# Tcadart/pyLatticeDSO

Hardware: AMD Instinct MI355X
Metric: beams/s assembly+PCG-solve (higher is better)
Workload: dtype f64

## Files before the change

### include/pylattice_hip.h

```cpp
#ifndef PYLATTICE_HIP_H
#define PYLATTICE_HIP_H

#include <stdint.h>

#ifdef __cplusplus
extern "C" {
#endif

typedef struct pl_context *pl_handle;

typedef enum {
  PL_OK = 0,
  PL_ERR_ARG = -1,
  PL_ERR_HIP = -2,
  PL_ERR_STATE = -3,
  PL_ERR_NOCONV = -4,
  PL_ERR_NAN = -5,
  PL_ERR_NODEVICE = -6
} pl_status;

typedef struct {
  int64_t n_nodes;
  int64_t n_beams;
  const double *node_xyz;
// ... 90 lines not shown
int pl_ddm_set_geometry(pl_handle h, const double *node_xyz );

int pl_set_bc(pl_handle h, const uint8_t *fixed, const double *ubar, const double *f);

int pl_set_periodic(pl_handle h, const int32_t *master );

int pl_update_radii(pl_handle h, const double *beam_radius);
int pl_set_multiplicity(pl_handle h, const double *beam_mult );
int pl_update_segments(pl_handle h, const double *seg_len, const int32_t *seg_nsub);

int pl_assemble(pl_handle h);

int pl_assemble_bsr(pl_handle h, int with_bc, int64_t *n_block_rows, int64_t *n_blocks);
int pl_get_bsr(pl_handle h, int64_t *rowptr , int32_t *colidx , double *vals );

int pl_spmv(pl_handle h, const double *x, double *y);
int pl_spmv_free(pl_handle h, const double *x, double *y);
int pl_spmv_bsr(pl_handle h, const double *x, double *y);

int pl_solve(pl_handle h, double rtol, int32_t max_iter, double *u, pl_stats_t *stats);

int pl_reactions(pl_handle h, const double *u, double *R);

int pl_sens(pl_handle h, const double *u, const double *lam, double *dCdr);

int pl_node_mod(pl_handle h, const double *u, double *out);

int pl_stress(pl_handle h, const double *u , int32_t where,
              double *station ,
              double *peak );
int pl_stress_pnorm(pl_handle h, const double *u , int32_t where, double p, double *phi, double *sigma_max,
                    double *dphi_du , double *dphi_dr );

int pl_buckling(pl_handle h, const double *u , int32_t length, double k_eff, int32_t shear,
                double *util , double *n_axial , double *n_crit );
int pl_buckling_pnorm(pl_handle h, const double *u , int32_t length, double k_eff, int32_t shear, double p,
                      double *bp, double *util_max, double *dbp_du , double *dbp_dr );

int pl_energy(pl_handle h, const double *u, double *energy);

int pl_schur(pl_handle h, const int32_t *boundary_nodes, int32_t nb, double rtol, int32_t max_iter, double *S);

#define PL_MULTI_MAX 64
int pl_spmv_multi(pl_handle h, int32_t n_rhs, int masked, const double *x, double *y);
int pl_solve_multi(pl_handle h, int32_t n_rhs, const double *ubar, const double *f, double rtol, int32_t max_iter,
                   double *u, pl_stats_t *stats);
int pl_schur_block(pl_handle h, const int32_t *boundary_nodes, int32_t nb, double rtol, int32_t max_iter,
                   int32_t block, double *S);

int pl_geom_spmv_multi(pl_handle h, const double *u, int32_t n_rhs, int masked, const double *x, double *y);
int pl_buckling_modes(pl_handle h, const double *u , int32_t n_modes, int32_t n_sub,
                      double rtol, int32_t max_iter,
                      double tol, int32_t max_outer,
                      double *load_factor , double *modes ,
                      double *residual ,
                      int32_t *n_found, int32_t *outer_iterations);

int pl_schur_cells(const pl_opts_t *o, int32_t n_inst, int32_t n_nodes, int32_t n_beams,
                   const int32_t *beam_conn , int32_t nb,
                   const int32_t *boundary_nodes ,
                   const double *node_xyz , const double *beam_radius ,
                   const double *seg_len , const int32_t *seg_nsub ,
                   double *S , int32_t *info );

int pl_cells_recover(const pl_opts_t *o, int32_t n_inst, int32_t n_nodes, int32_t n_beams,
                     const int32_t *beam_conn , int32_t nb,
                     const int32_t *boundary_nodes ,
                     const double *node_xyz , const double *beam_radius ,
                     const double *seg_len , const int32_t *seg_nsub ,
                     const double *u_b ,
                     const double *lam_b ,
                     double *u_full ,
                     double *lam_full ,
                     double *sens ,
                     int32_t *info );

int pl_get_records(pl_handle h, double *rec);

int pl_debug_partition(pl_handle h, int32_t *tile_of_node, int32_t *agg_of_node, int32_t *local_agg_of_node,
                       uint8_t *eliminated);

int pl_time_kernel(pl_handle h, int which, int reps, double *avg_ms);
int pl_algorithmic_bytes(pl_handle h, double *out3);
int pl_forget_history(pl_handle h);

int pl_debug_spd_solve(int device, int32_t n, const double *A, const double *b, double *x, double *quad,
                       int32_t fp32_factor);

int pl_dist_unique_id_bytes(void);
int pl_dist_unique_id(void *id_out);
int pl_dist_loopback_id(void *id_out);
int pl_dist_abort(pl_handle h);
int pl_dist_init(pl_handle h, int rank, int world, const void *unique_id, const int32_t *shared_local,
                 const int32_t *shared_global, int32_t n_shared, int32_t n_shared_global);

typedef struct pl_lattice pl_lattice;
typedef struct {
  int64_t n_nodes, n_beams, n_cell_beam, n_cell_node, n_created;
} pl_lattice_info_t;
int pl_generate_lattice(int64_t n_cells, const double *cell_coord, const double *cell_size, const double *cell_radii,
                        int32_t n_geom, int32_t n_tmpl, const double *tmpl, const int32_t *tmpl_type,
                        pl_lattice **out, pl_lattice_info_t *info);
int pl_lattice_fetch(const pl_lattice *L, double *node_xyz, int32_t *beam_conn, double *beam_radius, int32_t *beam_type,
                     int32_t *beam_cell0, int64_t *cell_beam_ptr , int64_t *cell_beam_idx,
                     int64_t *cell_node_ptr , int64_t *cell_node_idx, int32_t *created_nodes,
                     int32_t *created_beam);
void pl_lattice_free(pl_lattice *L);

int pl_penalize(int64_t n_beams, const double *node_xyz, const int32_t *beam_conn, const double *lzone ,
                double mesh_size, double *seg_len , int32_t *seg_nsub , double *pen_xyz );

int pl_boundary_index(int64_t n_cells, const int64_t *cell_node_ptr, const int64_t *cell_node_idx, int64_t n_nodes,
                      const double *node_xyz, const double *cell_coord, const double *cell_size, int64_t *index_boundary,
                      int64_t *visit, int64_t *n_visit);

int pl_boundary_index_rows(int64_t n_cells, const int64_t *cell_node_ptr, const int64_t *cell_node_idx, int64_t n_nodes,
                           const double *node_xyz, const double *cell_coord, const double *cell_size,
                           int64_t *index_boundary, int64_t *visit, int64_t *n_visit);

int pl_dist_set_peers(pl_handle h, const int32_t *shared_peer );

#ifdef __cplusplus
}
#endif
#endif
```

### pylatticedso_amd/_capi.py

```python
from __future__ import annotations

import ctypes as C
import os

import numpy as np

from .timing import timing as _timing

_HERE = os.path.dirname(os.path.abspath(__file__))
LIB_PATH = os.environ.get("PYLATTICE_HIP_LIB") or os.path.join(_HERE, "libpylattice_hip.so")

PL_OK, PL_ERR_ARG, PL_ERR_HIP, PL_ERR_STATE, PL_ERR_NOCONV, PL_ERR_NAN, PL_ERR_NODEVICE = 0, -1, -2, -3, -4, -5, -6

EXPORTS = ["pl_default_opts", "pl_opts_size", "pl_stats_size", "pl_abi_version", "pl_last_error", "pl_version", "pl_lzone", "pl_create", "pl_create_ddm",
           "pl_ddm_set_preconditioner", "pl_ddm_set_geometry", "pl_ddm_update_matrices", "pl_destroy", "pl_set_bc", "pl_set_periodic",
           "pl_update_radii", "pl_set_multiplicity", "pl_update_segments", "pl_assemble", "pl_assemble_bsr", "pl_get_bsr", "pl_spmv",
           "pl_spmv_free", "pl_spmv_bsr", "pl_solve", "pl_reactions", "pl_sens", "pl_energy", "pl_node_mod", "pl_schur",
           "pl_stress", "pl_stress_pnorm", "pl_buckling", "pl_buckling_pnorm",
           "pl_spmv_multi", "pl_solve_multi", "pl_schur_block", "pl_geom_spmv_multi", "pl_buckling_modes",
           "pl_schur_cells", "pl_cells_recover", "pl_get_records", "pl_debug_partition", "pl_time_kernel", "pl_algorithmic_bytes", "pl_forget_history", "pl_debug_spd_solve", "pl_dist_unique_id_bytes",
           "pl_dist_unique_id", "pl_dist_loopback_id", "pl_dist_abort", "pl_dist_init", "pl_dist_set_peers", "pl_generate_lattice", "pl_lattice_fetch",
           "pl_lattice_free", "pl_penalize", "pl_boundary_index", "pl_boundary_index_rows"]


class PlMesh(C.Structure):
    _fields_ = [("n_nodes", C.c_int64), ("n_beams", C.c_int64), ("node_xyz", C.c_void_p),
                ("beam_conn", C.c_void_p), ("beam_radius", C.c_void_p), ("seg_len", C.c_void_p),
                ("seg_nsub", C.c_void_p)]


class PlOpts(C.Structure):
    _fields_ = [("struct_size", C.c_uint32), ("abi_version", C.c_uint32),
                ("young", C.c_double), ("poisson", C.c_double), ("kappa", C.c_double), ("pen_coef", C.c_double),
                ("device", C.c_int32), ("spmv_kernel", C.c_int32), ("precond", C.c_int32), ("reorder", C.c_int32),
                ("check_every", C.c_int32), ("lanes_per_node", C.c_int32),
                ("tile_nodes", C.c_int32), ("coarse_max_dofs", C.c_int32), ("palette", C.c_int32),
                ("local_max_dofs", C.c_int32), ("precision", C.c_int32), ("restart_every", C.c_int32),
                ("alpha_max", C.c_double), ("grid_lo", C.c_double * 3), ("grid_hi", C.c_double * 3),
                ("grid_nodes", C.c_int64), ("mintol", C.c_double), ("compact_records", C.c_int32),
                ("condense", C.c_int32), ("chol_persistent", C.c_int32), ("cg_form", C.c_int32),
                ("tile_modes", C.c_int32), ("coarse_modes", C.c_int32), ("overlap", C.c_int32),
                ("coarse_storage", C.c_int32), ("warm_start", C.c_int32), ("short_iteration", C.c_int32)]


class PlStats(C.Structure):
    _fields_ = [("struct_size", C.c_uint32), ("iterations", C.c_int32), ("converged", C.c_int32),
                ("reserved_i", C.c_int32), ("rel_residual", C.c_double),
                ("b_norm", C.c_double), ("ms_assembly", C.c_double), ("ms_solve", C.c_double),
                ("ms_spmv_avg", C.c_double), ("precond_used", C.c_double), ("restarts", C.c_double),
                ("precision_used", C.c_double), ("info", C.c_double), ("stop_reason", C.c_double),
                ("condensed_nodes", C.c_double), ("cg_form_used", C.c_double), ("kp_form", C.c_double),
                ("comm_world", C.c_double), ("comm_rank", C.c_double), ("short_iteration_used", C.c_double),
                ("reserved", C.c_double * 2)]


class PlError(RuntimeError):
    def __init__(self, code, msg):
        super().__init__(f"libpylattice_hip error {code}: {msg}")
        self.code = code


_lib = None


def load_library(path: str | None = None):
    global _lib
    if _lib is not None and path is None:
        return _lib
    p = path or LIB_PATH
    if not os.path.exists(p):
        raise FileNotFoundError(f"{p} not found - build it with `make -C pylatticedso_amd/csrc` "
                                "(the HIP path has no CPU fallback)")
    lib = C.CDLL(p)
    lib.pl_last_error.restype = C.c_char_p
    lib.pl_version.restype = C.c_char_p
    lib.pl_destroy.restype = None
    for name in ("pl_opts_size", "pl_stats_size", "pl_abi_version"):
        getattr(lib, name).restype = C.c_uint32
    lib.pl_lattice_free.restype = None
    V, I32, I64, D = C.c_void_p, C.c_int32, C.c_int64, C.c_double
    sig = {"pl_default_opts": [V, C.c_uint32], "pl_opts_size": [], "pl_stats_size": [], "pl_abi_version": [], "pl_lzone": [I32, I64, I64, V, V, V, V], "pl_create": [V, V, V], "pl_create_ddm": [I64, I64, I32, V, I32, V, V, V, V],
           "pl_ddm_set_preconditioner": [V, I32, V, V], "pl_ddm_set_geometry": [V, V], "pl_ddm_update_matrices": [V, I32, V, V], "pl_destroy": [V], "pl_set_bc": [V, V, V, V], "pl_set_periodic": [V, V],
           "pl_update_radii": [V, V], "pl_set_multiplicity": [V, V], "pl_update_segments": [V, V, V], "pl_assemble": [V],
           "pl_assemble_bsr": [V, I32, V, V], "pl_get_bsr": [V, V, V, V], "pl_spmv": [V, V, V],
           "pl_spmv_free": [V, V, V], "pl_spmv_bsr": [V, V, V], "pl_solve": [V, D, I32, V, V],
           "pl_reactions": [V, V, V], "pl_sens": [V, V, V, V], "pl_energy": [V, V, V], "pl_node_mod": [V, V, V],
           "pl_stress": [V, V, I32, V, V], "pl_stress_pnorm": [V, V, I32, D, V, V, V, V],
           "pl_buckling": [V, V, I32, D, I32, V, V, V], "pl_buckling_pnorm": [V, V, I32, D, I32, D, V, V, V, V],
           "pl_schur": [V, V, I32, D, I32, V], "pl_spmv_multi": [V, I32, I32, V, V],
           "pl_solve_multi": [V, I32, V, V, D, I32, V, V], "pl_schur_block": [V, V, I32, D, I32, I32, V],
           "pl_geom_spmv_multi": [V, V, I32, I32, V, V],
           "pl_buckling_modes": [V, V, I32, I32, D, I32, D, I32, V, V, V, V, V],
           "pl_schur_cells": [V, I32, I32, I32, V, I32, V, V, V, V, V, V, V],
           "pl_cells_recover": [V, I32, I32, I32, V, I32, V, V, V, V, V, V, V, V, V, V, V],
           "pl_get_records": [V, V], "pl_debug_partition": [V, V, V, V, V], "pl_time_kernel": [V, I32, I32, V],
           "pl_algorithmic_bytes": [V, V], "pl_forget_history": [V], "pl_debug_spd_solve": [I32, I32, V, V, V, V, I32], "pl_dist_unique_id_bytes": [], "pl_dist_unique_id": [V], "pl_dist_loopback_id": [V], "pl_dist_abort": [V],
           "pl_dist_init": [V, I32, I32, V, V, V, I32, I32], "pl_dist_set_peers": [V, V],
           "pl_generate_lattice": [I64, V, V, V, I32, I32, V, V, V, V], "pl_lattice_fetch": [V] * 12,
           "pl_lattice_free": [V], "pl_penalize": [I64, V, V, V, D, V, V, V],
           "pl_boundary_index": [I64, V, V, I64, V, V, V, V, V, V],
           "pl_boundary_index_rows": [I64, V, V, I64, V, V, V, V, V, V]}
    for name, args in sig.items():
        getattr(lib, name).argtypes = args
    if lib.pl_opts_size() != C.sizeof(PlOpts) or lib.pl_stats_size() != C.sizeof(PlStats):
        raise ImportError(f"{p}: pl_opts_t / pl_stats_t are {lib.pl_opts_size()} / {lib.pl_stats_size()} bytes in the "
                          f"library, {C.sizeof(PlOpts)} / {C.sizeof(PlStats)} in this binding (ABI version "
                          f"{lib.pl_abi_version()}): rebuild libpylattice_hip.so")
    _lib = lib
    return lib


def default_opts(lib=None) -> "PlOpts":
    lib = lib or load_library()
    opts = PlOpts()
    _check(lib, lib.pl_default_opts(C.byref(opts), C.sizeof(PlOpts)))
    return opts


def _ptr(a):
    return None if a is None else a.ctypes.data_as(C.c_void_p)


def _f64(a, n=None):
    a = np.ascontiguousarray(a, dtype=np.float64)
    if n is not None and a.size != n:
        raise ValueError(f"expected {n} values, got {a.size}")
    return a


def _check(lib, rc, allow=()):
    if rc != PL_OK and rc not in allow:
        raise PlError(rc, lib.pl_last_error().decode())
    return rc


def lzone(node_xyz, beam_conn, beam_radius, device=0):
    lib = load_library()
    xyz = _f64(np.asarray(node_xyz).reshape(-1))
    conn = np.ascontiguousarray(beam_conn, dtype=np.int32).reshape(-1)
    rad = _f64(np.asarray(beam_radius).reshape(-1), len(conn) // 2)
    out = np.empty(len(conn), np.float64)
    _check(lib, lib.pl_lzone(int(device), len(xyz) // 3, len(conn) // 2, _ptr(xyz), _ptr(conn), _ptr(rad), _ptr(out)))
    return out.reshape(-1, 2)


def debug_spd_solve(A, b, device=0, fp32_factor=False):
    lib = load_library()
    A = np.ascontiguousarray(A, np.float64)
    b = np.ascontiguousarray(b, np.float64)
    x = np.empty_like(b)
    q = C.c_double()
    _check(lib, lib.pl_debug_spd_solve(device, len(b), _ptr(A), _ptr(b), _ptr(x), C.byref(q), int(bool(fp32_factor))))
    return x, q.value


MULTI_MAX = 64

SCHUR_CELLS_MAX_BOUNDARY, SCHUR_CELLS_MAX_INTERIOR, SCHUR_CELLS_MAX_BEAMS = 32, 16, 512


def schur_cells_fits(n_nodes, n_beams, n_boundary):
    return (0 < n_boundary <= SCHUR_CELLS_MAX_BOUNDARY and n_nodes - n_boundary <= SCHUR_CELLS_MAX_INTERIOR
            and 0 < n_beams <= SCHUR_CELLS_MAX_BEAMS)


def _per_instance(name, a, tail, n_inst):
    if a.shape == tail:
        a = np.broadcast_to(a, (n_inst,) + tail)
    elif a.shape != (n_inst,) + tail:
        raise ValueError(f"{name} must have shape {tail} or {(n_inst,) + tail}, got {a.shape}")
    return np.ascontiguousarray(a)


def schur_cells(node_xyz, beam_conn, boundary_nodes, beam_radius, seg_len, seg_nsub, young, poisson, kappa=0.9,
                pen_coef=1.5, device=0, n_inst=None):
    xyz, conn, bn, rad, slen, nsub, n_inst = _cell_batch_arrays(node_xyz, beam_conn, boundary_nodes, beam_radius, seg_len,
                                                                seg_nsub, n_inst)
    B, N = len(conn), xyz.shape[1]
    lib = load_library()
# ... 440 lines not shown
        return S

    def _columns(self, name, a, k=None):
        n6 = 6 * self.n_nodes
        a = np.asarray(a, dtype=np.float64)
        if a.shape in ((self.n_nodes, 6), (n6,)):
            a = a.reshape(1, n6)
        elif a.ndim == 3 and a.shape[1:] == (self.n_nodes, 6):
            a = a.reshape(a.shape[0], n6)
        elif not (a.ndim == 2 and a.shape[1] == n6):
            raise ValueError(f"{name} must have shape (k, {self.n_nodes}, 6) or (k, {n6}), got {a.shape}")
        if not 1 <= a.shape[0] <= MULTI_MAX:
            raise ValueError(f"{name}: 1 ... {MULTI_MAX} columns per call, got {a.shape[0]}")
        if k is not None and a.shape[0] != k:
            raise ValueError(f"{name} has {a.shape[0]} columns, {k} expected")
        return np.ascontiguousarray(a)

    def spmv_multi(self, X, masked=False):
        x = self._columns("X", X)
        y = np.empty_like(x)
        _check(self._lib, self._lib.pl_spmv_multi(self._h, x.shape[0], int(bool(masked)), _ptr(x), _ptr(y)))
        return y.reshape(x.shape[0], self.n_nodes, 6)

    def solve_multi(self, ubar=None, f=None, rtol=1e-8, max_iter=20000, raise_on_noconv=True):
        if ubar is None and f is None:
            raise ValueError("solve_multi needs ubar or f (they give the number of columns)")
        ub = None if ubar is None else self._columns("ubar", ubar)
        ff = None if f is None else self._columns("f", f, None if ub is None else ub.shape[0])
        k = (ub if ub is not None else ff).shape[0]
        u = np.empty((k, 6 * self.n_nodes), np.float64)
        st = (PlStats * k)()
        for s in st:
            s.struct_size = C.sizeof(PlStats)
        rc = self._lib.pl_solve_multi(self._h, k, _ptr(ub), _ptr(ff), float(rtol), int(max_iter), _ptr(u), st)
        keys = [n for n, _ in PlStats._fields_ if n not in ("reserved", "reserved_i", "struct_size")]
        stats = [{n: getattr(s, n) for n in keys} for s in st]
        if rc in (PL_OK, PL_ERR_NOCONV):
            _timing.device("pl_solve_multi: PCG (HIP events)", st[0].ms_solve)
        _check(self._lib, rc, allow=() if raise_on_noconv else (PL_ERR_NOCONV,))
        return u.reshape(k, self.n_nodes, 6), stats

    def geom_spmv_multi(self, X, u=None, masked=False):
        x = self._columns("X", X)
        u = None if u is None else _f64(np.asarray(u).reshape(-1), 6 * self.n_nodes)
        y = np.empty_like(x)
        _check(self._lib, self._lib.pl_geom_spmv_multi(self._h, _ptr(u), x.shape[0], int(bool(masked)), _ptr(x), _ptr(y)))
        return y.reshape(x.shape[0], self.n_nodes, 6)

    def buckling_modes(self, n_modes=4, u=None, n_sub=0, rtol=1e-10, max_iter=200000, tol=1e-9, max_outer=200,
                       raise_on_noconv=True):
        u = None if u is None else _f64(np.asarray(u).reshape(-1), 6 * self.n_nodes)
        n_modes = int(n_modes)
        lam = np.empty(max(n_modes, 0), np.float64)
        modes = np.empty((max(n_modes, 0), self.n_nodes, 6), np.float64)
        res = np.empty(max(n_modes, 0), np.float64)
        found, outer = C.c_int32(), C.c_int32()
        rc = self._lib.pl_buckling_modes(self._h, _ptr(u), n_modes, int(n_sub), float(rtol), int(max_iter), float(tol),
                                         int(max_outer), _ptr(lam), _ptr(modes), _ptr(res), C.byref(found), C.byref(outer))
        _check(self._lib, rc, allow=() if raise_on_noconv else (PL_ERR_NOCONV,))
        return {"load_factor": lam, "modes": modes, "residual": res, "n_found": found.value,
                "outer_iterations": outer.value}

    def geom_spmv_multi_host(self, X, u, masked=False, fixed=None):
        from . import geometric_host as GH
        if masked and fixed is None:
            raise ValueError("the masked product needs the mask given to set_bc")
        x = self._columns("X", X).reshape(-1, self.n_nodes, 6)
        return GH.geometric_apply(self.records(), self.beam_conn, u, x, fixed if masked else None)

    def buckling_modes_host(self, u, fixed, n_modes=4, n_sub=0, tol=1e-9, max_outer=200, dense=False):
        from . import geometric_host as GH
        rec = self.records()
        K = GH.elastic_matrix(rec, self.beam_conn, self.n_nodes)
        Kg = GH.geometric_matrix(rec, self.beam_conn, u, self.n_nodes)
        if dense:
            return GH.buckling_modes_dense(K, Kg, fixed, n_modes)
        return GH.buckling_modes_subspace(K, Kg, fixed, n_modes, n_sub, tol, max_outer)

    def time_kernel(self, which, reps=20):
        ms = C.c_double()
        _check(self._lib, self._lib.pl_time_kernel(self._h, int(which), int(reps), C.byref(ms)))
        return ms.value

    def algorithmic_bytes(self):
        out = (C.c_double * 3)()
        _check(self._lib, self._lib.pl_algorithmic_bytes(self._h, out))
        return {"spmv": out[0], "pcg_iter": out[1], "bsr": out[2]}

    def set_periodic(self, master):
        m = None if master is None else np.ascontiguousarray(master, dtype=np.int32)
        if m is not None and m.size != self.n_nodes:
            raise ValueError(f"expected {self.n_nodes} entries, got {m.size}")
        _check(self._lib, self._lib.pl_set_periodic(self._h, _ptr(m)))

    def forget_history(self):
        _check(self._lib, self._lib.pl_forget_history(self._h))

    @staticmethod
    def dist_unique_id() -> bytes:
        lib = load_library()
        n = lib.pl_dist_unique_id_bytes()
        buf = C.create_string_buffer(n)
        _check(lib, lib.pl_dist_unique_id(buf))
        return buf.raw

    @staticmethod
    def dist_loopback_id() -> bytes:
        lib = load_library()
        buf = C.create_string_buffer(lib.pl_dist_unique_id_bytes())
        _check(lib, lib.pl_dist_loopback_id(buf))
        return buf.raw

    def dist_abort(self):
        if getattr(self, "_h", None) is not None and self._h.value:
            self._lib.pl_dist_abort(self._h)

    def dist_init(self, rank, world, unique_id: bytes, shared_local, shared_global, n_shared_global, shared_peer=None):
        sl = np.ascontiguousarray(shared_local, dtype=np.int32)
        sg = np.ascontiguousarray(shared_global, dtype=np.int32)
        buf = C.create_string_buffer(unique_id, len(unique_id))
        _check(self._lib, self._lib.pl_dist_init(self._h, int(rank), int(world), buf, _ptr(sl), _ptr(sg),
                                                 int(len(sl)), int(n_shared_global)))
        if shared_peer is not None:
            sp = np.ascontiguousarray(shared_peer, dtype=np.int32)
            if sp.shape != sl.shape:
                raise ValueError("one peer rank per shared entry expected")
            _check(self._lib, self._lib.pl_dist_set_peers(self._h, _ptr(sp)))


for _name in ("assemble", "assemble_bsr", "get_bsr", "solve", "set_bc", "spmv", "spmv_free", "spmv_bsr", "reactions",
              "sens", "stress", "stress_pnorm", "buckling", "buckling_pnorm", "energy", "schur", "spmv_multi", "solve_multi", "geom_spmv_multi", "buckling_modes", "update_radii", "update_segments", "records"):
    _f = getattr(HipLattice, _name, None)
    if _f is not None:
        _f._timing_category = "hip"
        setattr(HipLattice, _name, _timing.timeit(_f))
```

### pylatticedso_amd/csrc/pl_api.hip

```cpp
#include "pl_solver.h"
#include "pl_condense.h"
#include "pl_multi.h"
#include "pl_stress.h"
#include "pl_buckling.h"
#include "pl_geom.h"


namespace {
template <typename WT>
int debug_spd_solve_t(int device, int32_t n, const double *A, const double *b, double *x, double *quad) {
  if (n <= 0 || !A || !b || !x) return fail(PL_ERR_ARG, "pl_debug_spd_solve: bad argument");
  int ndev = 0;
  if (hipGetDeviceCount(&ndev) != hipSuccess || ndev <= 0) return fail(PL_ERR_NODEVICE, "no HIP device visible");
  PL_HIP(hipSetDevice(device));
  const int np = (n + pl::kNB - 1) / pl::kNB * pl::kNB;
  std::vector<double> Ap((size_t)np * np, 0.0), bp(np, 0.0);
  for (int i = 0; i < np; ++i) {
    if (i < n) {
      std::memcpy(&Ap[(size_t)i * np], A + (size_t)i * n, n * sizeof(double));
      bp[i] = b[i];
    } else {
      Ap[(size_t)i * np + i] = 1.0;
    }
  }
// ... 756 lines not shown
    const size_t nn = (size_t)np * np;
    PL_HIP(h->dd_A.alloc(nn));
    PL_HIP(h->dd_Lf.alloc(nn));
    PL_HIP(h->dd_W.alloc(nn));
    PL_HIP(h->dd_Wt.alloc(nn));
    PL_HIP(h->dd_Dinv.alloc((size_t)np * pl::kNB));
    PL_HIP(h->dd_tv.alloc(np));
    PL_HIP(h->dd_info.alloc(2));
    PL_HIP(hipMemsetAsync(h->dd_W.p, 0, nn * sizeof(double), h->stream));
    PL_HIP(hipMemsetAsync(h->dd_Wt.p, 0, nn * sizeof(double), h->stream));
    h->dd_n = np;
  }
  h->dd_ready = false;
  PL_HIP(hipMemsetAsync(h->dd_A.p, 0, (size_t)np * np * sizeof(double), h->stream));
  PL_HIP(hipMemsetAsync(h->dd_info.p, 0, 2 * sizeof(int), h->stream));
  const int m = 6 * h->ddm_nb;
  const int64_t ne = h->ddm_cells * m * m;
  const uint8_t *fx = h->have_bc ? h->fixed.p : (const uint8_t *)nullptr;
  hipLaunchKernelGGL(pl::k_ddm_dense_assemble, dim3(grid_for(ne)), dim3(pl::kBlock), 0, h->stream, h->ddm_cells,
                     h->ddm_nb, h->ddm_cell_nodes.p, h->ddm_have_P ? h->ddm_cell_P.p : h->ddm_cell_S.p,
                     h->ddm_have_P ? h->ddm_Pt.p : h->ddm_St.p, fx, np, h->dd_A.p);
  hipLaunchKernelGGL(pl::k_ddm_dense_unit, dim3((np + 255) / 256), dim3(256), 0, h->stream, n6, np, fx, h->dd_A.p);
  pl::dense_factor_inverse(h->dd_A.p, h->dd_Lf.p, h->dd_W.p, h->dd_Wt.p, h->dd_Dinv.p, np, np, h->dd_info.p,
                           h->dd_bw, h->stream);
  PL_HIP(hipGetLastError());
  int info[2] = {0, 0};
  PL_HIP(hipMemcpyAsync(info, h->dd_info.p, sizeof(info), hipMemcpyDeviceToHost, h->stream));
  PL_HIP(hipStreamSynchronize(h->stream));
  h->dd_ready = (info[0] == 0);
  return PL_OK;
}

static int fem_factor_dense(pl_context *h) {
  const int64_t n6 = h->N * 6;
  const int np = (int)((n6 + pl::kNB - 1) / pl::kNB * pl::kNB);
  if (h->dd_n != np) {
    const size_t nn = (size_t)np * np;
    PL_HIP(h->dd_A.alloc(nn));
    PL_HIP(h->dd_Lf.alloc(nn));
    PL_HIP(h->dd_W.alloc(nn));
    PL_HIP(h->dd_Wt.alloc(nn));
    PL_HIP(h->dd_Dinv.alloc((size_t)np * pl::kNB));
    PL_HIP(h->dd_tv.alloc(np));
    PL_HIP(h->dd_info.alloc(2));
    PL_HIP(hipMemsetAsync(h->dd_W.p, 0, nn * sizeof(double), h->stream));
    PL_HIP(hipMemsetAsync(h->dd_Wt.p, 0, nn * sizeof(double), h->stream));
    h->dd_n = np;
    int64_t band = 0;
    for (int64_t i = 0; i < h->N; ++i)
      for (int64_t q = h->h_rowptr[i]; q < h->h_rowptr[i + 1]; ++q) band = std::max<int64_t>(band, std::llabs((long long)(h->h_col[q] - i)));
    h->dd_bw = (int)((6 * (band + 1) + pl::kNB - 1) / pl::kNB + 1);
  }
  h->dd_ready = false;
  int rc = ensure_bsr_buffers(h);
  if (rc) return rc;
  PL_HIP(hipMemsetAsync(h->dd_A.p, 0, (size_t)np * np * sizeof(double), h->stream));
  PL_HIP(hipMemsetAsync(h->dd_info.p, 0, 2 * sizeof(int), h->stream));
  rc = launch_bsr_fill(h, 1, h->stream);
  if (rc) return rc;
  h->have_bsr = false;
  hipLaunchKernelGGL(pl::k_bsr_to_dense, dim3(grid_for(h->nblk * 36)), dim3(pl::kBlock), 0, h->stream, h->N, h->nblk,
                     h->bsr_rowptr.p, h->bsr_col.p, (const double *)h->bsr_vals.p, np, h->dd_A.p);
  hipLaunchKernelGGL(pl::k_ddm_dense_unit, dim3((np + 255) / 256), dim3(256), 0, h->stream, n6, np, (const uint8_t *)nullptr,
                     h->dd_A.p);
  pl::dense_factor_inverse(h->dd_A.p, h->dd_Lf.p, h->dd_W.p, h->dd_Wt.p, h->dd_Dinv.p, np, np, h->dd_info.p, h->dd_bw,
                           h->stream);
  PL_HIP(hipGetLastError());
  int info[2] = {0, 0};
  PL_HIP(hipMemcpyAsync(info, h->dd_info.p, sizeof(info), hipMemcpyDeviceToHost, h->stream));
  PL_HIP(hipStreamSynchronize(h->stream));
  h->dd_ready = (info[0] == 0);
  if (h->dd_ready) PL_HIP(hipMemsetAsync(h->dinv.p, 0, n6 * sizeof(double), h->stream));
  return PL_OK;
}

void pl_destroy(pl_handle h) {
  if (!h) return;
  (void)hipSetDevice(h->opt.device);
  (void)hipStreamSynchronize(h->stream);
  if (h->comm_stream) (void)hipStreamSynchronize(h->comm_stream);
  pl::dist_destroy(h->dist);
  if (h->pal_host_flags != h->pal_fallback_flags) (void)hipHostFree(h->pal_host_flags);
  if (h->cls_host_flag) (void)hipHostFree(h->cls_host_flag);
  delete h;
}

int pl_set_bc(pl_handle h, const uint8_t *fixed, const double *ubar, const double *f) {
  if (!valid(h) || !fixed) return fail(PL_ERR_ARG, "pl_set_bc: null argument");
  PL_HIP(hipSetDevice(h->opt.device));
  const int64_t N = h->N;
  const size_t n6 = (size_t)N * 6;
  std::vector<uint8_t> fx(n6), bits(N);
  double *st = nullptr;
  if (int rcs = staging(h, &st)) return rcs;
  pl::parallel_for(N, [&](int64_t i0, int64_t i1, unsigned) {
    for (int64_t i = i0; i < i1; ++i) {
      const size_t src = 6 * (size_t)h->perm[i];
      uint8_t b = 0;
      for (int k = 0; k < 6; ++k) {
        const uint8_t v = fixed[src + k] ? 1 : 0;
        fx[6 * i + k] = v;
        b |= (uint8_t)(v << k);
        st[6 * i + k] = (ubar && v) ? ubar[src + k] : 0.0;
      }
      bits[i] = b;
    }
  }, 1 << 15);
  PL_HIP(hipMemcpyAsync(h->ubar.p, st, n6 * sizeof(double), hipMemcpyHostToDevice, h->stream));
  PL_HIP(hipMemcpyAsync(h->fixed.p, fx.data(), n6, hipMemcpyHostToDevice, h->stream));
  PL_HIP(hipMemcpyAsync(h->fixedbits.p, bits.data(), N, hipMemcpyHostToDevice, h->stream));
  PL_HIP(hipStreamSynchronize(h->stream));
  pl::parallel_for(N, [&](int64_t i0, int64_t i1, unsigned) {
    for (int64_t i = i0; i < i1; ++i) {
      const size_t src = 6 * (size_t)h->perm[i];
      for (int k = 0; k < 6; ++k) st[6 * i + k] = f ? f[src + k] : 0.0;
    }
  }, 1 << 15);
  PL_HIP(hipMemcpyAsync(h->f.p, st, n6 * sizeof(double), hipMemcpyHostToDevice, h->stream));
  PL_HIP(hipStreamSynchronize(h->stream));
  const bool same_mask = h->have_bc && !h->dist.active && h->h_fixedbits == bits;
  h->h_fixedbits = bits;
  if (same_mask) return PL_OK;
  h->have_bc = true;
  h->coarse.n_fix = -1;
  h->coarseL.n_fix = -1;
  {
    int rcs = select_condensed(h, bits);
    if (rcs) return rcs;
  }
  if (h->assembled && h->opkind == 1) {
    if (h->opt.precond >= 2 && h->opt.precond <= 4) {
      h->assembled = false;
      h->dd_ready = false;
      h->dd_blocks = false;
      h->dd2_ready = false;
    } else {
      pl::launch_invert_diag(h->N * 6, h->diag.p, h->fixed.p, h->dinv.p, h->stream);
      PL_HIP(hipStreamSynchronize(h->stream));
    }
  } else if (h->assembled) {
    int rc = launch_diag(h, h->stream);
    if (rc) return rc;
    rc = finish_diag_dist(h);
    if (rc) return rc;
    rc = launch_local_mask(h);
    if (rc) return rc;
    rc = launch_tile_blocks(h, h->stream);
    if (rc) return rc;
    rc = build_coarse(h);
    if (rc) return rc;
    rc = launch_dinv32(h);
    if (rc) return rc;
    rc = agree_condensed(h);
    if (rc) return rc;
    rc = launch_condensed_blocks(h, h->stream);
    if (rc) return rc;
    PL_HIP(hipStreamSynchronize(h->stream));
    {
      const bool keep = h->pal_ready;
      finish_condensed_classes(h);
      (void)keep;
    }
    if (h->bsr_with_bc) h->have_bsr = false;
    if (h->opt.precond == 5 && !h->dist.active) {
      rc = fem_factor_dense(h);
      if (rc) return rc;
    }
  }
  return PL_OK;
}

int pl_set_periodic(pl_handle h, const int32_t *master) {
  if (!valid(h)) return fail(PL_ERR_ARG, "pl_set_periodic: null handle");
  if (h->opkind != 0) return fail(PL_ERR_STATE, "pl_set_periodic: not available on a DDM handle");
  h->n_per_groups = 0;
  if (!master) return PL_OK;
  if (h->opt.precond != 1 || h->dist.active)
    return fail(PL_ERR_STATE, "pl_set_periodic: periodic constraints are served by the Jacobi PCG of a single-GPU handle (opts.precond = 1)");
  PL_HIP(hipSetDevice(h->opt.device));
  const int64_t N = h->N;
  std::vector<int32_t> inv((size_t)N);
  for (int64_t i = 0; i < N; ++i) inv[(size_t)h->perm[i]] = (int32_t)i;
  std::vector<int32_t> cnt((size_t)N, 0);
  for (int64_t i = 0; i < N; ++i) {
    const int32_t m = master[i];
    if (m < 0 || m >= N || master[m] != m) return fail(PL_ERR_ARG, "pl_set_periodic: master[i] must name a node that is its own master");
    cnt[(size_t)m]++;
  }
  std::vector<int32_t> ptr(1, 0), nodes, start((size_t)N, -1);
  for (int64_t m = 0; m < N; ++m)
    if (cnt[(size_t)m] >= 2) {
      start[(size_t)m] = (int32_t)ptr.size() - 1;
      ptr.push_back(ptr.back() + cnt[(size_t)m]);
    }
  nodes.resize((size_t)ptr.back());
  std::vector<int32_t> fill(ptr.begin(), ptr.end() - 1);
  for (int64_t i = 0; i < N; ++i) {
    const int32_t g = start[(size_t)master[i]];
    if (g >= 0) nodes[(size_t)fill[(size_t)g]++] = inv[(size_t)i];
  }
  const int64_t ng = (int64_t)ptr.size() - 1;
  if (ng == 0) return PL_OK;
  PL_HIP(h->per_ptr.alloc(ptr.size()));
  PL_HIP(h->per_nodes.alloc(nodes.size()));
  PL_HIP(hipMemcpy(h->per_ptr.p, ptr.data(), ptr.size() * sizeof(int32_t), hipMemcpyHostToDevice));
  PL_HIP(hipMemcpy(h->per_nodes.p, nodes.data(), nodes.size() * sizeof(int32_t), hipMemcpyHostToDevice));
  h->n_per_groups = ng;
  return PL_OK;
}

int pl_update_radii(pl_handle h, const double *beam_radius) {
  if (!valid(h) || !beam_radius) return fail(PL_ERR_ARG, "pl_update_radii: null argument");
  if (h->opkind != 0) return fail(PL_ERR_STATE, "pl_update_radii: not available on a DDM handle");
  for (int64_t b = 0; b < h->B; ++b)
    if (!(beam_radius[b] > 0.0)) return fail(PL_ERR_ARG, "pl_update_radii: non-positive radius");
  PL_HIP(hipSetDevice(h->opt.device));
  double *stg = nullptr;
  int rc = stagingB(h, &stg);
  if (rc) return rc;
  pl::parallel_for(h->B, [&](int64_t b0, int64_t b1, unsigned) {
    for (int64_t b = b0; b < b1; ++b) stg[b] = beam_radius[h->bperm[b]];
  }, 1 << 16);
  PL_HIP(hipMemcpyAsync(h->radius.p, stg, h->B * sizeof(double), hipMemcpyHostToDevice, h->stream));
  PL_HIP(hipStreamSynchronize(h->stream));
  h->assembled = false;
  h->have_bsr = false;
  return PL_OK;
}

int pl_set_multiplicity(pl_handle h, const double *beam_mult) {
  if (!valid(h)) return fail(PL_ERR_ARG, "pl_set_multiplicity: null handle");
  if (h->opkind != 0) return fail(PL_ERR_STATE, "pl_set_multiplicity: not available on a DDM handle");
  PL_HIP(hipSetDevice(h->opt.device));
  if (!beam_mult) {
    h->mult.release();
  } else {
    for (int64_t b = 0; b < h->B; ++b)
      if (!(beam_mult[b] > 0.0)) return fail(PL_ERR_ARG, "pl_set_multiplicity: non-positive multiplicity");
    std::vector<double> m(h->B);
    for (int64_t b = 0; b < h->B; ++b) m[b] = beam_mult[h->bperm[b]];
    if (!h->mult.p) PL_HIP(h->mult.alloc(h->B));
    PL_HIP(hipMemcpy(h->mult.p, m.data(), h->B * sizeof(double), hipMemcpyHostToDevice));
  }
  h->assembled = false;
  h->have_bsr = false;
  return PL_OK;
}

int pl_update_segments(pl_handle h, const double *seg_len, const int32_t *seg_nsub) {
  if (!valid(h) || !seg_len || !seg_nsub) return fail(PL_ERR_ARG, "pl_update_segments: null argument");
  PL_HIP(hipSetDevice(h->opt.device));
  std::vector<double> sl((size_t)h->B * 3);
  std::vector<int32_t> sn((size_t)h->B * 3);
  for (int64_t b = 0; b < h->B; ++b)
    for (int k = 0; k < 3; ++k) {
      sl[3 * b + k] = seg_len[3 * (size_t)h->bperm[b] + k];
      sn[3 * b + k] = seg_nsub[3 * (size_t)h->bperm[b] + k];
    }
  PL_HIP(hipMemcpy(h->seg_len.p, sl.data(), 3 * h->B * sizeof(double), hipMemcpyHostToDevice));
  PL_HIP(hipMemcpy(h->seg_nsub.p, sn.data(), 3 * h->B * sizeof(int32_t), hipMemcpyHostToDevice));
  h->assembled = false;
  h->have_bsr = false;
  return PL_OK;
}

int pl_assemble(pl_handle h) {
  if (!valid(h)) return fail(PL_ERR_ARG, "pl_assemble: null handle");
  PL_HIP(hipSetDevice(h->opt.device));
  if (h->opkind == 1) {
    if (h->assembled && (h->opt.precond == 0 || (h->opt.precond == 1 && !h->dd_ready && !h->dd_blocks) || h->dd_ready || h->dd_blocks)) {
      h->ms_assembly = 0.0;
      return PL_OK;
    }
    h->dd_ready = false;
    h->dd_blocks = false;
    h->dd2_ready = false;
    if (h->opt.precond == 4 && !h->dd2_plan)
      return fail(PL_ERR_STATE, "pl_assemble: precond = 4 on a DDM handle needs the node positions (pl_ddm_set_geometry)");
    if (h->opt.precond == 3 || h->opt.precond == 4) {
      PL_HIP(hipEventRecord(h->ev0, h->stream));
      if (!h->dd_B.p) PL_HIP(h->dd_B.alloc((size_t)h->N * 36));
      PL_HIP(hipMemsetAsync(h->dd_B.p, 0, (size_t)h->N * 36 * sizeof(double), h->stream));
      const int64_t ne = (int64_t)h->ddm_cells * h->ddm_nb * 36;
      hipLaunchKernelGGL(pl::k_ddm_node_blocks, dim3(grid_for(ne)), dim3(pl::kBlock), 0, h->stream, h->ddm_cells, h->ddm_nb,
                         h->ddm_cell_nodes.p, h->ddm_have_P ? h->ddm_cell_P.p : h->ddm_cell_S.p,
                         h->ddm_have_P ? h->ddm_Pt.p : h->ddm_St.p, h->dd_B.p);
      hipLaunchKernelGGL(pl::k_ddm_node_blocks_invert, dim3(grid_for(h->N)), dim3(pl::kBlock), 0, h->stream, h->N,
                         h->have_bc ? (const uint8_t *)h->fixed.p : (const uint8_t *)nullptr, h->dd_B.p);
      PL_HIP(hipMemsetAsync(h->dinv.p, 0, h->N * 6 * sizeof(double), h->stream));
      int info2[2] = {0, 0};
      if (h->opt.precond == 4) {
        pl::Coarse &cs = h->dd2;
        const int n = cs.ncp, m = 6 * h->ddm_nb;
        PL_HIP(hipMemsetAsync(cs.Ac, 0, (size_t)n * n * sizeof(double), h->stream));
        PL_HIP(hipMemsetAsync(cs.info, 0, 2 * sizeof(int), h->stream));
        hipLaunchKernelGGL(pl::k_ddm_coarse_cells, dim3((unsigned)h->ddm_cells), dim3(pl::kWave),
                           (size_t)2 * m * pl::kDdmModes * sizeof(double), h->stream, h->ddm_cells, h->ddm_nb,
                           h->ddm_cell_nodes.p, h->ddm_have_P ? h->ddm_cell_P.p : h->ddm_cell_S.p,
                           h->ddm_have_P ? h->ddm_Pt.p : h->ddm_St.p, h->dd2_agg.p, h->dd2_cen.p, h->dd2_xyz.p,
                           h->have_bc ? (const uint8_t *)h->fixed.p : (const uint8_t *)nullptr, n, cs.Ac);
        hipLaunchKernelGGL(pl::k_coarse_regularize, dim3((n + 255) / 256), dim3(256), 0, h->stream, n, cs.Ac);
        pl::TrtriPhases ph;
        ph.rows = 3;
        ph.stream = h->side2;
        ph.ev_go = h->ev_t0;
        ph.ev_done = h->ev_t1;
        pl::coarse_factor(cs, n, h->stream, nullptr, (unsigned *)nullptr, ph);
        cs.ainv_ready = false;
        if (cs.Ainv) {
          const long tiles = (long)(n / 32) * (n / 32 + 1) / 2;
          if (cs.w16)
            hipLaunchKernelGGL(pl::k_dense_explicit_inverse<pl::bf16_t>, dim3((unsigned)((tiles + 3) / 4)), dim3(256), 0,
                               h->stream, n, reinterpret_cast<const pl::bf16_t *>(cs.W), n, cs.Ainv);
          else
            hipLaunchKernelGGL(pl::k_dense_explicit_inverse<float>, dim3((unsigned)((tiles + 3) / 4)), dim3(256), 0, h->stream,
                               n, (const float *)cs.W, n, cs.Ainv);
          cs.ainv_ready = true;
        }
        PL_HIP(hipMemcpyAsync(info2, cs.info, sizeof(info2), hipMemcpyDeviceToHost, h->stream));
      }
      PL_HIP(hipEventRecord(h->ev1, h->stream));
      PL_HIP(hipEventSynchronize(h->ev1));
      PL_HIP(hipGetLastError());
      float ms = 0.f;
      PL_HIP(hipEventElapsedTime(&ms, h->ev0, h->ev1));
      h->ms_assembly = ms;
      h->dd2_ready = h->opt.precond == 4 && info2[0] == 0;
      h->dd_blocks = true;
      h->assembled = true;
      return PL_OK;
    }
    if (h->opt.precond == 2) {
      PL_HIP(hipEventRecord(h->ev0, h->stream));
      int rcp = ddm_factor_preconditioner(h);
      if (rcp) return rcp;
      if (h->dd_ready) {
        PL_HIP(hipMemsetAsync(h->dinv.p, 0, h->N * 6 * sizeof(double), h->stream));
        PL_HIP(hipEventRecord(h->ev1, h->stream));
        PL_HIP(hipEventSynchronize(h->ev1));
        float ms = 0.f;
        PL_HIP(hipEventElapsedTime(&ms, h->ev0, h->ev1));
        h->ms_assembly = ms;
        h->assembled = true;
        return PL_OK;
      }
    }
    if (h->opt.precond >= 1) {
      PL_HIP(hipMemsetAsync(h->diag.p, 0, h->N * 6 * sizeof(double), h->stream));
      const int64_t m = (int64_t)h->ddm_cells * h->ddm_nb * 6;
      hipLaunchKernelGGL(pl::k_ddm_diag, dim3(grid_for(m)), dim3(pl::kBlock), 0, h->stream, h->ddm_cells, h->ddm_nb,
                         h->ddm_cell_nodes.p, h->ddm_cell_S.p, h->ddm_St.p, h->diag.p);
    } else {
      pl::launch_fill(h->N * 6, 1.0, h->diag.p, h->stream);
    }
    pl::launch_invert_diag(h->N * 6, h->diag.p, h->have_bc ? h->fixed.p : nullptr, h->dinv.p, h->stream);
    PL_HIP(hipStreamSynchronize(h->stream));
    h->ms_assembly = 0.0;
    h->assembled = true;
    return PL_OK;
  }
  int rc = agree_condensed(h);
  if (rc) return rc;
  PL_HIP(hipEventRecord(h->ev0, h->stream));
  rc = launch_records(h);
  if (rc) return rc;
  rc = launch_local_mask(h);
  if (rc) return rc;
  PL_HIP(hipEventRecord(h->ev_fork, h->stream));
  PL_HIP(hipStreamWaitEvent(h->side, h->ev_fork, 0));
  rc = launch_palette(h, h->side);
  if (rc) return rc;
  rc = launch_diag(h, h->dist.active ? h->stream : h->side);
  if (rc) return rc;
  rc = finish_diag_dist(h);
  if (rc) return rc;
  rc = launch_tile_blocks(h, h->side);
  if (rc) return rc;
  rc = launch_condensed_blocks(h, h->side);
  if (rc) return rc;
  const bool refresh_bsr = h->want_bsr && (!h->bsr_with_bc || h->have_bc);
  int rc_fill = PL_OK;
  bool fill_queued = false;
  int64_t split = 0;
  if (refresh_bsr && h->side_cu && h->coarse.enabled && h->have_bc) {
    static const double kChainLinkMs = [] { const char *e = std::getenv("PL_CHAIN_LINK_MS"); return e ? std::atof(e) : 0.04; }();
    static const double kFillBlocksPerMs = [] { const char *e = std::getenv("PL_FILL_BLOCKS_PER_MS"); return e ? std::atof(e) : 8.5e6; }();
    const double chain_ms = kChainLinkMs * std::max(0, h->coarse.ncp / pl::kNB - 1);
    const double fit = chain_ms * kFillBlocksPerMs / std::max<double>(1.0, (double)h->nblk);
    split = fit >= 1.0 ? h->n_slices : (int64_t)(fit * (double)h->n_slices);
    if (split < h->n_slices / 16) split = 0;
  }
  bool part1_queued = false;
  auto queue_fill = [&](int phase) {
    if (!refresh_bsr || fill_queued) return;
    if (phase == 0) {
      if (split <= 0 || part1_queued) return;
      part1_queued = true;
      if (hipEventRecord(h->ev_chol, h->stream) != hipSuccess || hipStreamWaitEvent(h->side_cu, h->ev_chol, 0) != hipSuccess ||
          hipStreamWaitEvent(h->side_cu, h->ev_join, 0) != hipSuccess) {
        rc_fill = fail(PL_ERR_HIP, "pl_assemble: could not order the BSR fill beside the factorisation");
        return;
      }
      rc_fill = launch_bsr_fill(h, h->bsr_with_bc, h->side_cu, 0, split);
      if (hipEventRecord(h->ev_fill1, h->side_cu) != hipSuccess) rc_fill = fail(PL_ERR_HIP, "pl_assemble: event record failed");
      return;
    }
    fill_queued = true;
    if (hipEventRecord(h->ev_chol, h->stream) != hipSuccess || hipStreamWaitEvent(h->side, h->ev_chol, 0) != hipSuccess) {
      rc_fill = fail(PL_ERR_HIP, "pl_assemble: could not order the BSR fill behind the factorisation");
      return;
    }
    if (!rc_fill) rc_fill = launch_bsr_fill(h, h->bsr_with_bc, h->side, part1_queued ? split : 0, -1);
    if (part1_queued && hipStreamWaitEvent(h->side, h->ev_fill1, 0) != hipSuccess)
      rc_fill = fail(PL_ERR_HIP, "pl_assemble: event wait failed");
    if (hipEventRecord(h->ev_join, h->side) != hipSuccess) rc_fill = fail(PL_ERR_HIP, "pl_assemble: event record failed");
  };
  PL_HIP(hipEventRecord(h->ev_join, h->side));
  h->dd_ready = false;
  if (h->opt.precond == 5 && h->have_bc && !h->dist.active) {
    PL_HIP(hipStreamWaitEvent(h->stream, h->ev_join, 0));
    rc = fem_factor_dense(h);
    if (rc) return rc;
  }
  rc = build_coarse(h, h->coarse.enabled && h->have_bc ? std::function<void(int)>(queue_fill) : std::function<void(int)>());
  if (rc) return rc;
  queue_fill(1);
  if (rc_fill) return rc_fill;
  PL_HIP(hipStreamWaitEvent(h->stream, h->ev_join, 0));
  rc = launch_dinv32(h);
  if (rc) return rc;
  PL_HIP(hipEventRecord(h->ev1, h->stream));
  PL_HIP(hipStreamSynchronize(h->stream));
  finish_palette(h);
  finish_condensed_classes(h);
  for (pl::Coarse *cs : {&h->coarse, &h->coarseL})
    if (cs->ready && cs->Ac) {
      PL_HIP(hipMemsetAsync(cs->Ac, 0, (size_t)cs->ncp * cs->ncp * sizeof(double), h->stream));
      cs->ac_clean = true;
    }
  float ms = 0.f;
  PL_HIP(hipEventElapsedTime(&ms, h->ev0, h->ev1));
  h->ms_assembly = ms;
  h->assembled = true;
  h->have_bsr = refresh_bsr;
  return PL_OK;
}

int pl_assemble_bsr(pl_handle h, int with_bc, int64_t *n_block_rows, int64_t *n_blocks) {
  if (!valid(h)) return fail(PL_ERR_ARG, "pl_assemble_bsr: null handle");
  if (h->opkind != 0) return fail(PL_ERR_STATE, "pl_assemble_bsr: not available on a DDM handle");
  if (!h->assembled) return fail(PL_ERR_STATE, "pl_assemble_bsr: call pl_assemble first");
  if (with_bc && !h->have_bc) return fail(PL_ERR_STATE, "pl_assemble_bsr: with_bc needs pl_set_bc");
  PL_HIP(hipSetDevice(h->opt.device));
  if (int rcb = ensure_bsr_buffers(h)) return rcb;
  const bool fresh = h->have_bsr && h->want_bsr && h->bsr_with_bc == (with_bc ? 1 : 0);
  h->want_bsr = true;
  h->bsr_with_bc = with_bc ? 1 : 0;
  if (fresh) {
    if (n_block_rows) *n_block_rows = h->N;
    if (n_blocks) *n_blocks = h->nblk;
    return PL_OK;
  }
  PL_HIP(hipEventRecord(h->ev0, h->stream));
  int rc = launch_bsr_fill(h, with_bc, h->stream);
  if (rc) return rc;
  PL_HIP(hipEventRecord(h->ev1, h->stream));
  PL_HIP(hipStreamSynchronize(h->stream));
  float ms = 0.f;
  PL_HIP(hipEventElapsedTime(&ms, h->ev0, h->ev1));
  h->ms_assembly += ms;
  h->have_bsr = true;
  if (n_block_rows) *n_block_rows = h->N;
  if (n_blocks) *n_blocks = h->nblk;
  return PL_OK;
}

int pl_get_bsr(pl_handle h, int64_t *rowptr, int32_t *colidx, double *vals) {
  if (!valid(h)) return fail(PL_ERR_ARG, "pl_get_bsr: null handle");
  if (!h->have_bsr) return fail(PL_ERR_STATE, "pl_get_bsr: call pl_assemble_bsr first");
  PL_HIP(hipSetDevice(h->opt.device));
  std::vector<double> v((size_t)h->nblk * 36);
  PL_HIP(hipMemcpy(v.data(), h->bsr_vals.p, v.size() * sizeof(double), hipMemcpyDeviceToHost));
  if (!h->reordered) {
    if (rowptr) std::memcpy(rowptr, h->h_rowptr.data(), (h->N + 1) * sizeof(int64_t));
    if (colidx) std::memcpy(colidx, h->h_col.data(), h->nblk * sizeof(int32_t));
    if (vals) std::memcpy(vals, v.data(), v.size() * sizeof(double));
    return PL_OK;
  }
  std::vector<int64_t> rp(h->N + 1, 0);
  for (int64_t ci = 0; ci < h->N; ++ci) {
    const int64_t di = h->iperm[ci];
    rp[ci + 1] = rp[ci] + (h->h_rowptr[di + 1] - h->h_rowptr[di]);
  }
  if (rowptr) std::memcpy(rowptr, rp.data(), (h->N + 1) * sizeof(int64_t));
  std::vector<std::pair<int32_t, int64_t>> row;
  for (int64_t ci = 0; ci < h->N; ++ci) {
    const int64_t di = h->iperm[ci];
    row.clear();
    for (int64_t p = h->h_rowptr[di]; p < h->h_rowptr[di + 1]; ++p) row.push_back({h->perm[h->h_col[p]], p});
    std::stable_sort(row.begin(), row.end(), [](auto &l, auto &r) { return l.first < r.first; });
    for (size_t k = 0; k < row.size(); ++k) {
      if (colidx) colidx[rp[ci] + k] = row[k].first;
      if (vals) std::memcpy(vals + 36 * (rp[ci] + k), &v[36 * row[k].second], 36 * sizeof(double));
    }
  }
  return PL_OK;
}

static int spmv_common(pl_handle h, const double *x, double *y, bool masked, const char *who) {
  if (!valid(h) || !x || !y) return fail(PL_ERR_ARG, std::string(who) + ": null argument");
  if (!h->assembled) return fail(PL_ERR_STATE, std::string(who) + ": call pl_assemble first");
  if (masked && !h->have_bc) return fail(PL_ERR_STATE, std::string(who) + ": call pl_set_bc first");
  PL_HIP(hipSetDevice(h->opt.device));
  std::vector<double> stage;
  int rc = upload6(h, x, h->tmp.p, stage);
  if (rc) return rc;
  if (masked) {
// ... 1056 lines not shown
      case 0: return launch_spmv(h, h->p.p, h->Ap.p, true, h->scal.p + pl::S_PAP * pl::kSlots);
      case 1: {
        int r1 = launch_records(h);
        return r1 ? r1 : build_palette(h);
      }
      case 2: return launch_bsr_fill(h, 0, h->stream);
      case 3: return pcg_iteration(h, k);
      case 4:
        hipLaunchKernelGGL(pl::k_bsr_spmv, dim3(grid_for(h->N)), dim3(pl::kBlock), 0, h->stream, h->N,
                           h->bsr_rowptr.p, h->bsr_col.p, h->bsr_vals.p, h->p.p, h->Ap.p);
        return PL_OK;
      case 5:
        if (!h->dist.active) return fail(PL_ERR_STATE, "pl_time_kernel: 5/6 need pl_dist_init");
        return pl::dist_sum_shared(h->dist, h->Ap.p, h->stream, h->scal.p + pl::S_PAP * pl::kSlots, pl::kSlots)
                   ? fail(PL_ERR_HIP, "RCCL all-reduce failed") : PL_OK;
      case 6:
        if (!h->dist.active || !h->coarse.ready) return fail(PL_ERR_STATE, "pl_time_kernel: 6 needs a coarse level");
        return pl::dist_sum_scalars(h->dist, h->coarse.tv, h->coarse.ncp, h->stream)
                   ? fail(PL_ERR_HIP, "RCCL all-reduce failed") : PL_OK;
      case 7:
      case 8:
      case 9: {
        if (!(h->coarse.ready && h->tile.ready && choose_kernel(h) == 3))
          return fail(PL_ERR_STATE, "pl_time_kernel: 7/8/9 need the multi-level PCG on the tile kernel");
        float *p32 = reinterpret_cast<float *>(h->z.p), *Ap32 = p32 + n6;
        double *cur = h->scal.p + (k & 1) * pl::S_COUNT * pl::kSlots, *nxt = h->scal.p + ((k + 1) & 1) * pl::S_COUNT * pl::kSlots;
        int r7 = launch_spmv_f32(h, p32, Ap32, true, cur + pl::S_PAP * pl::kSlots);
        if (r7 || which == 7) return r7;
        if (which == 8) {
          float *x32 = reinterpret_cast<float *>(h->tmp.p), *r32 = x32 + n6;
          return pcg_tail_coarse_t<float, float>(h, cur, nxt, k, p32, (const float *)Ap32, x32, r32);
        }
        return pcg_tail_coarse_t<float, double>(h, cur, nxt, k, p32, (const float *)Ap32, h->x.p, h->r.p);
      }
      case 10: {
        if (mp_applies(h)) {
          float *p32 = reinterpret_cast<float *>(h->z.p), *Ap32 = p32 + n6;
          if (h->cond_use) {
            int r0 = launch_spmv_f32(h, p32, p32, false, nullptr, nullptr, pl::kEndsCondensedSolve);
            return r0 ? r0 : launch_spmv_f32(h, p32, Ap32, true, h->scal.p + pl::S_PAP * pl::kSlots, h->maskC.p, pl::kEndsOthers);
          }
          return launch_spmv_f32(h, p32, Ap32, true, h->scal.p + pl::S_PAP * pl::kSlots);
        }
        if (h->cond_use) {
          int r0 = launch_spmv(h, h->p.p, h->p.p, false, nullptr, nullptr, pl::kEndsCondensedSolve);
          return r0 ? r0 : launch_spmv(h, h->p.p, h->Ap.p, true, h->scal.p + pl::S_PAP * pl::kSlots, h->maskC.p, pl::kEndsOthers);
        }
        return launch_spmv(h, h->p.p, h->Ap.p, true, h->scal.p + pl::S_PAP * pl::kSlots);
      }
      case 11: {
        if (!(mp_applies(h) && h->opt.precision == 1)) return pcg_iteration(h, k);
        float *p32 = reinterpret_cast<float *>(h->z.p), *Ap32 = p32 + n6;
        float *x32 = reinterpret_cast<float *>(h->tmp.p), *r32 = x32 + n6;
        double *cur = h->scal.p + (k & 1) * pl::S_COUNT * pl::kSlots, *nxt = h->scal.p + ((k + 1) & 1) * pl::S_COUNT * pl::kSlots;
        int r11;
        if (h->cond_use) {
          r11 = launch_spmv_f32(h, p32, p32, false, nullptr, nullptr, pl::kEndsCondensedSolve);
          if (!r11) r11 = launch_spmv_f32(h, p32, Ap32, true, cur + pl::S_PAP * pl::kSlots, h->maskC.p, pl::kEndsOthers);
        } else {
          r11 = launch_spmv_f32(h, p32, Ap32, true, cur + pl::S_PAP * pl::kSlots);
        }
        return r11 ? r11 : pcg_tail_coarse_t<float, float>(h, cur, nxt, k, p32, (const float *)Ap32, x32, r32);
      }
      default: return fail(PL_ERR_ARG, "pl_time_kernel: unknown kernel id");
    }
  };
  for (int k = 0; k < 3; ++k) {
    rc = one(0);
    if (rc) return rc;
  }
  PL_HIP(hipEventRecord(h->ev0, h->stream));
  for (int k = 0; k < reps; ++k) {
    rc = one(k);
    if (rc) return rc;
  }
  PL_HIP(hipEventRecord(h->ev1, h->stream));
  PL_HIP(hipStreamSynchronize(h->stream));
  float ms = 0.f;
  PL_HIP(hipEventElapsedTime(&ms, h->ev0, h->ev1));
  *avg_ms = (double)ms / reps;
  return PL_OK;
}

int pl_debug_spd_solve(int device, int32_t n, const double *A, const double *b, double *x, double *quad,
                       int32_t fp32_factor) {
  return fp32_factor ? debug_spd_solve_t<float>(device, n, A, b, x, quad)
                     : debug_spd_solve_t<double>(device, n, A, b, x, quad);
}

int pl_lzone(int device, int64_t n_nodes, int64_t n_beams, const double *node_xyz, const int32_t *beam_conn,
             const double *beam_radius, double *lzone) {
  if (n_nodes <= 0 || n_beams <= 0 || !node_xyz || !beam_conn || !beam_radius || !lzone)
    return fail(PL_ERR_ARG, "pl_lzone: bad argument");
  int ndev = 0;
  if (hipGetDeviceCount(&ndev) != hipSuccess || ndev <= 0)
    return fail(PL_ERR_NODEVICE, "pl_lzone: no HIP device visible (libpylattice_hip has no CPU fallback)");
  if (device < 0 || device >= ndev) return fail(PL_ERR_ARG, "pl_lzone: bad device ordinal");
  const int64_t nh = 2 * n_beams;
  std::vector<int64_t> ptr((size_t)n_nodes + 1, 0);
  for (int64_t h = 0; h < nh; ++h) {
    const int32_t v = beam_conn[h];
    if (v < 0 || v >= n_nodes) return fail(PL_ERR_ARG, "pl_lzone: node id out of range");
    ptr[(size_t)v + 1]++;
  }
  for (int64_t i = 0; i < n_nodes; ++i) ptr[i + 1] += ptr[i];
  std::vector<int32_t> half((size_t)nh);
  {
    std::vector<int64_t> fill(ptr.begin(), ptr.end() - 1);
    for (int64_t h = 0; h < nh; ++h) half[(size_t)fill[beam_conn[h]]++] = (int32_t)h;
  }
  PL_HIP(hipSetDevice(device));
  DevBuf<double> dx, dr, dl;
  DevBuf<int32_t> dc, dh;
  DevBuf<int64_t> dp;
  PL_HIP(dx.alloc((size_t)n_nodes * 3));
  PL_HIP(dr.alloc(n_beams));
  PL_HIP(dl.alloc(nh));
  PL_HIP(dc.alloc(nh));
  PL_HIP(dh.alloc(nh));
  PL_HIP(dp.alloc(n_nodes + 1));
  PL_HIP(hipMemcpy(dx.p, node_xyz, (size_t)n_nodes * 3 * sizeof(double), hipMemcpyHostToDevice));
  PL_HIP(hipMemcpy(dr.p, beam_radius, n_beams * sizeof(double), hipMemcpyHostToDevice));
  PL_HIP(hipMemcpy(dc.p, beam_conn, nh * sizeof(int32_t), hipMemcpyHostToDevice));
  PL_HIP(hipMemcpy(dh.p, half.data(), nh * sizeof(int32_t), hipMemcpyHostToDevice));
  PL_HIP(hipMemcpy(dp.p, ptr.data(), (n_nodes + 1) * sizeof(int64_t), hipMemcpyHostToDevice));
  hipLaunchKernelGGL(pl::k_lzone, dim3(grid_for(nh)), dim3(pl::kBlock), 0, nullptr, nh, dx.p, dc.p, dr.p, dp.p, dh.p,
                     dl.p);
  PL_HIP(hipGetLastError());
  PL_HIP(hipMemcpy(lzone, dl.p, nh * sizeof(double), hipMemcpyDeviceToHost));
  return PL_OK;
}

#ifdef PL_TILE_STAMPS
int pl_debug_tile_stamps(unsigned long long *out) {
  return hipMemcpyFromSymbol(out, HIP_SYMBOL(pl::g_tile_stamps), sizeof(unsigned long long) * 8 * 4096) == hipSuccess ? 0 : -2;
}
#endif

int pl_dist_unique_id_bytes(void) { return pl::dist_unique_id_bytes(); }
int pl_dist_unique_id(void *id_out) {
  if (!id_out) return fail(PL_ERR_ARG, "pl_dist_unique_id: null argument");
  return pl::dist_unique_id(id_out) ? fail(PL_ERR_HIP, "ncclGetUniqueId failed") : PL_OK;
}
int pl_dist_loopback_id(void *id_out) {
  if (!id_out) return fail(PL_ERR_ARG, "pl_dist_loopback_id: null argument");
  pl::dist_loopback_id(id_out);
  return PL_OK;
}
int pl_dist_init(pl_handle h, int rank, int world, const void *unique_id, const int32_t *shared_local,
                 const int32_t *shared_global, int32_t n_shared, int32_t n_shared_global) {
  if (!valid(h) || !unique_id || world < 1 || rank < 0 || rank >= world || n_shared < 0)
    return fail(PL_ERR_ARG, "pl_dist_init: bad argument");
  if (n_shared > 0 && (!shared_local || !shared_global)) return fail(PL_ERR_ARG, "pl_dist_init: null index array");
  PL_HIP(hipSetDevice(h->opt.device));
  std::vector<int32_t> loc(n_shared);
  for (int i = 0; i < n_shared; ++i) {
    if (shared_local[i] < 0 || shared_local[i] >= h->N || shared_global[i] < 0 || shared_global[i] >= n_shared_global)
      return fail(PL_ERR_ARG, "pl_dist_init: shared node index out of range");
    loc[i] = h->iperm[shared_local[i]];
  }
  int rc = pl::dist_init(h->dist, rank, world, unique_id, loc.data(), shared_global, n_shared, n_shared_global, h->N,
                         h->stream);
  if (rc == 6)
    return fail(PL_ERR_ARG, "pl_dist_init: loopback group mismatch (all ranks of a loopback id must share one device and one "
                            "world size <= " + std::to_string(pl::kLoopMaxWorld) + ", each rank attaches once)");
  if (rc) return fail(PL_ERR_HIP, "pl_dist_init: communicator setup failed (" + std::to_string(rc) + ")");
// ... 62 lines not shown
```

### pylatticedso_amd/csrc/pl_assembly.h

```cpp
#pragma once
#include "pl_ops.h"

namespace {

inline bool small_wanted(const pl_context *c) {
  const pl::Coarse &cs = c->coarse;
  if (c->opt.short_iteration < 0 || c->opkind != 0 || c->dist.active || c->coarseL.enabled || c->opt.precision != 0 ||
      c->opt.cg_form == 1 || !cs.enabled || !c->tile.ready || choose_kernel(c) != 3 || c->opt.mintol > 0.0 ||
      c->opt.restart_every > 0)
    return false;
  if (c->opt.short_iteration == 1) return true;
  static const double auto_mb = [] { const char *e = std::getenv("PL_SHORT_ITERATION_MB"); return e ? std::atof(e) : 16.0; }();
  return (double)cs.n_tiles * cs.cm * cs.ncp * 4.0 <= auto_mb * 1048576.0;
}


int launch_records(pl_context *c) {
  hipLaunchKernelGGL(pl::k_build_records, dim3(grid_for(c->B)), dim3(pl::kBlock), 0, c->stream, c->B, c->xyz.p,
                     c->conn.p, c->radius.p, c->seg_len.p, c->seg_nsub.p, c->mult.p, c->mat, c->rec.p, c->rec5.p);
  PL_HIP(hipGetLastError());
  return PL_OK;
}

void refresh_visit_words(pl_context *c, hipStream_t st) {
// ... 54 lines not shown
  PL_HIP(hipMemsetAsync(c->pal_keys.p, 0xFF, pl::kPalSize * sizeof(unsigned long long), st));
  PL_HIP(hipMemsetAsync(c->pal_owner.p, 0x7F, pl::kPalSize * sizeof(int), st));
  PL_HIP(hipMemsetAsync(c->pal_flags.p, 0, 2 * sizeof(int), st));
  PL_HIP(hipMemsetAsync(c->palette.p, 0, pl::kPalSize * sizeof(pl::Record), st));
  const dim3 g(grid_for(c->B)), blk(pl::kBlock);
  hipLaunchKernelGGL(pl::k_pal_insert, g, blk, 0, st, c->B, c->rec.p, c->pal_keys.p, c->pal_owner.p, c->pal_id.p,
                     c->pal_flags.p);
  hipLaunchKernelGGL(pl::k_pal_publish, g, blk, 0, st, c->B, c->rec.p, c->pal_owner.p, c->pal_id.p, c->palette.p);
  hipLaunchKernelGGL(pl::k_pal_verify, g, blk, 0, st, c->B, c->rec.p, c->pal_id.p, c->palette.p, c->pal_owner.p,
                     c->pal_flags.p, c->pal_dense_of_slot.p, c->pal_dense.p, pl::kPalDenseMax);
  refresh_visit_words(c, st);
  if (c->pal_dense2.p)
    hipLaunchKernelGGL(pl::k_pal_orient, dim3(1), dim3(pl::kPalDenseMax), 0, st, pl::kPalDenseMax, c->pal_dense.p,
                       c->pal_dense2.p);
  PL_HIP(hipGetLastError());
  PL_HIP(hipMemcpyAsync(c->pal_host_flags, c->pal_flags.p, 2 * sizeof(int), hipMemcpyDeviceToHost, st));
  return PL_OK;
}
void finish_palette(pl_context *c) {
  if (!c->opt.palette) return;
  if (c->pal_skipped) {
    c->pal_entries = 0;
    c->pal_ready = false;
    c->pal_lds = false;
    c->pal_rows = false;
    return;
  }
  c->pal_entries = c->pal_host_flags[1];
  c->pal_ready = (c->pal_host_flags[0] == 0);
  static const bool lds_off = [] { const char *e = std::getenv("PL_TILE_LDS"); return e && e[0] == '0'; }();
  c->pal_lds = c->pal_ready && c->vword.p && c->pal_entries > 0 && c->pal_entries <= pl::kPalDenseMax && !lds_off;
  if (c->pal_ready && !c->pal_lds && !lds_off && small_wanted(c) && c->rec5.p && c->vword_dir.p && c->tile.n_dir > 0 &&
      c->tile.n_dir <= pl::kPalDenseMax)
    c->pal_ready = false;
  if (c->pal_ready) {
    c->pal_fail_streak = 0;
  } else {
    c->pal_fail_streak = std::min(c->pal_fail_streak + 1, 4);
    c->pal_skip_left = (1 << c->pal_fail_streak) - 1;
  }
  const char *re = std::getenv("PL_ROWS");
  c->pal_rows = c->pal_lds && c->rword.p && c->pal_dense2.p && re && re[0] == '1';
}
int build_palette(pl_context *c) {
  int rc = launch_palette(c, c->stream);
  if (rc) return rc;
  PL_HIP(hipStreamSynchronize(c->stream));
  finish_palette(c);
  return PL_OK;
}

int launch_diag(pl_context *c, hipStream_t st) {
  const unsigned g = grid_for(c->n_slices, pl::kBlock / pl::kWave);
  const uint8_t *fb = c->have_bc ? c->fixedbits.p : (const uint8_t *)nullptr;
#define PL_D(L)                                                                                                  \
  hipLaunchKernelGGL((pl::k_diag_gather<L>), dim3(g), dim3(pl::kBlock), 0, st, c->N, c->slice_ptr.p, c->ent.p, \
                     c->rec.p, fb, c->diag.p, c->dinv.p)
  switch (c->lpn) { case 1: PL_D(1); break; case 2: PL_D(2); break; case 4: PL_D(4); break; case 8: PL_D(8); break;
                    default: PL_D(16); }
#undef PL_D
  PL_HIP(hipGetLastError());
  return PL_OK;
}
int finish_diag_dist(pl_context *c) {
  if (!c->dist.active) return PL_OK;
  int rc = pl::dist_sum_shared(c->dist, c->diag.p, c->stream);
  if (rc) return fail(PL_ERR_HIP, "RCCL all-reduce of the Jacobi diagonal failed");
  pl::launch_invert_diag(c->N * 6, c->diag.p, c->have_bc ? c->fixed.p : nullptr, c->dinv.p, c->stream);
  return PL_OK;
}

__global__ void k_local_mask(int64_t N, const uint8_t *__restrict__ fixedbits, const uint8_t *__restrict__ shared,
                             uint8_t *__restrict__ mask) {
  const int64_t i = (int64_t)blockIdx.x * blockDim.x + threadIdx.x;
  if (i < N) mask[i] = (uint8_t)(fixedbits[i] | (shared[i] ? 0x3f : 0));
}

int launch_dinv32(pl_context *c) {
  if (!c->coarse.enabled) return PL_OK;
  hipLaunchKernelGGL(pl::k_to_float, dim3(grid_for(c->N * 6)), dim3(pl::kBlock), 0, c->stream, c->N * 6, c->dinv.p,
                     c->coarse.dinv32);
  PL_HIP(hipGetLastError());
  return PL_OK;
}

int launch_local_mask(pl_context *c) {
  if (!c->coarse.enabled || !(c->dist.active || c->coarseL.enabled)) return PL_OK;
  hipLaunchKernelGGL(k_local_mask, dim3(grid_for(c->N)), dim3(pl::kBlock), 0, c->stream, c->N, c->fixedbits.p,
                     c->sharedbits.p, c->maskL.p);
  PL_HIP(hipGetLastError());
  return PL_OK;
}

inline int tile_modes_now(const pl_context *c) {
  return (c->coarse.tile_level && c->coarse.tile_modes == 12 && !c->coarseL.enabled) ? 12 : 6;
}

int launch_tile_blocks(pl_context *c, hipStream_t st) {
  pl::Coarse &cs = c->coarse;
  if (!cs.enabled || !c->have_bc || !cs.tile_level) return PL_OK;
  if (cs.cm == 12) return PL_OK;
  const uint8_t *fb = c->dist.active ? c->maskL.p : c->fixedbits.p;
  const bool twelve = tile_modes_now(c) == 12;
  if (!twelve)
    hipLaunchKernelGGL(pl::k_tile_blocks, dim3((unsigned)cs.n_tiles), dim3(pl::kBlock), 0, st, c->tile.tile_start.p,
                       c->tile.home_ptr.p, c->tile.foreign_ptr.p, c->tile.foreign_idx.p,
                       reinterpret_cast<const int2 *>(c->conn.p), c->rec.p, cs.agg_of_tile.p, cs.cen.p, c->xyz.p,
                       fb, cs.Bt_inv, (double *)nullptr);
  if (twelve) {
    hipLaunchKernelGGL(pl::k_tile_blocks_strain<true>, dim3((unsigned)cs.n_tiles), dim3(pl::kBlock), 0, st,
                       c->tile.tile_start.p, c->tile.home_ptr.p, c->tile.foreign_ptr.p, c->tile.foreign_idx.p,
                       reinterpret_cast<const int2 *>(c->conn.p), c->rec.p, cs.agg_of_tile.p, cs.cen.p, c->xyz.p, fb,
                       cs.Bt_raw);
    hipLaunchKernelGGL(pl::k_tile_blocks_strain<false>, dim3((unsigned)cs.n_tiles), dim3(pl::kBlock), 0, st,
                       c->tile.tile_start.p, c->tile.home_ptr.p, c->tile.foreign_ptr.p, c->tile.foreign_idx.p,
                       reinterpret_cast<const int2 *>(c->conn.p), c->rec.p, cs.agg_of_tile.p, cs.cen.p, c->xyz.p, fb,
                       cs.Bt_raw);
    hipLaunchKernelGGL(pl::k_tile_invert12, dim3((unsigned)cs.n_tiles), dim3(pl::kInv12Block), 0, st, cs.n_tiles,
                       (const double *)cs.Bt_raw, cs.Bt_inv);
  }
  PL_HIP(hipGetLastError());
  return PL_OK;
}

int build_coarse_level(pl_context *c, pl::Coarse &cs, const uint8_t *mask, bool reduce,
                       const std::function<void(int)> &after_chol = nullptr) {
  cs.ready = false;
  if (!cs.enabled || !c->have_bc) {
    if (after_chol) after_chol(1);
    return PL_OK;
  }
  bool tile_invert_pending = false;
  const int n = cs.ncp;
  if (!cs.ac_clean) PL_HIP(hipMemsetAsync(cs.Ac, 0, (size_t)n * n * sizeof(double), c->stream));
  cs.ac_clean = false;
  PL_HIP(hipMemsetAsync(cs.info, 0, 2 * sizeof(int), c->stream));
  if (cs.cm == 12) {
    const dim3 gt((unsigned)cs.n_tiles), blk(pl::kBlock);
    const int2 *conn2 = reinterpret_cast<const int2 *>(c->conn.p);
    const bool two_sets = c->dist.active;
    if (two_sets) {
      if (!cs.Bt_rawA && hipMalloc((void **)&cs.Bt_rawA, (size_t)cs.n_tiles * 144 * sizeof(double)) != hipSuccess)
        return fail(PL_ERR_HIP, "pl_assemble: out of device memory for the tile blocks");
      hipLaunchKernelGGL(pl::k_tile_blocks_strain<true>, gt, blk, 0, c->stream, c->tile.tile_start.p, c->tile.home_ptr.p,
                         c->tile.foreign_ptr.p, c->tile.foreign_idx.p, conn2, c->rec.p, cs.agg_of_tile.p, cs.cen.p,
                         c->xyz.p, (const uint8_t *)c->maskL.p, cs.Bt_raw);
      hipLaunchKernelGGL(pl::k_tile_blocks_strain<false>, gt, blk, 0, c->stream, c->tile.tile_start.p, c->tile.home_ptr.p,
                         c->tile.foreign_ptr.p, c->tile.foreign_idx.p, conn2, c->rec.p, cs.agg_of_tile.p, cs.cen.p,
                         c->xyz.p, (const uint8_t *)c->maskL.p, cs.Bt_raw);
    }
    double *rawA = two_sets ? cs.Bt_rawA : cs.Bt_raw;
    PL_HIP(hipEventRecord(c->ev_t0, c->stream));
    PL_HIP(hipStreamWaitEvent(c->side2, c->ev_t0, 0));
    hipLaunchKernelGGL(pl::k_tile_blocks_strain<true>, gt, blk, 0, c->side2, c->tile.tile_start.p, c->tile.home_ptr.p,
                       c->tile.foreign_ptr.p, c->tile.foreign_idx.p, conn2, c->rec.p, cs.agg_of_tile.p, cs.cen.p, c->xyz.p,
                       mask, rawA);
    if (cs.n_cross > 0)
      hipLaunchKernelGGL(pl::k_coarse_cross12, dim3(grid_for(cs.n_cross)), blk, 0, c->side2, cs.n_cross,
                         cs.cross_idx.p, c->conn.p, c->rec.p, cs.agg_of_node.p, cs.cen.p, c->xyz.p, mask, n, cs.Ac);
    PL_HIP(hipEventRecord(c->ev_t1, c->side2));
    hipLaunchKernelGGL(pl::k_tile_blocks_strain<false>, gt, blk, 0, c->stream, c->tile.tile_start.p, c->tile.home_ptr.p,
                       c->tile.foreign_ptr.p, c->tile.foreign_idx.p, conn2, c->rec.p, cs.agg_of_tile.p, cs.cen.p, c->xyz.p,
                       mask, rawA);
    PL_HIP(hipStreamWaitEvent(c->stream, c->ev_t1, 0));
    hipLaunchKernelGGL(pl::k_agg_add_tiles, dim3(grid_for(cs.n_tiles * 144)), blk, 0, c->stream, cs.n_tiles,
                       cs.agg_of_tile.p, (const double *)rawA, n, cs.Ac);
// ... 325 lines not shown
```

### pylatticedso_amd/csrc/pl_coarse.h

```cpp
#pragma once
#include <hip/hip_runtime.h>

#include <algorithm>
#include <cstdint>
#include <vector>

#include "pl_dense.h"
#include "pl_kernels.h"
#include "pl_tile.h"

namespace pl {


struct Coarse {
  bool enabled = false;
  bool ready = false;
  int n_agg = 0, nc = 0, ncp = 0;
  int cm = 6;
  int bw_blocks = 0;
  int64_t n_tiles = 0;
  int vblock = kBlock;
  TBuf<int32_t> agg_of_node, agg_of_tile;
  TBuf<int32_t> tile_of_node;
  TBuf<double> cen;
  TBuf<int32_t> cross_idx;
  int64_t n_cross = 0;
  float *Ainv = nullptr;
  bool ainv_ready = false;
  float *W = nullptr, *Wt = nullptr;
  bool w16 = false;
  double *Ac = nullptr, *Lf = nullptr, *Dinv = nullptr, *rc = nullptr, *yc = nullptr, *tv = nullptr;
  int *info = nullptr;
  unsigned *bar = nullptr;
  bool ac_clean = false;
  bool tile_level = true;
  std::vector<int32_t> h_tile_start;
  double *Bt_inv = nullptr, *yt = nullptr;
  int tile_modes = 6;
  double *Bt_raw = nullptr;
  double *Bt_rawA = nullptr;
  float *dinv32 = nullptr;
  TBuf<float> rel32;
  bool rel_exact = false;
  TBuf<int32_t> fix_list;
  int *fix_count = nullptr;
  int64_t n_fix = -1;
  ~Coarse() {
    for (void *q : {(void *)Ac, (void *)Lf, (void *)W, (void *)Wt, (void *)Dinv, (void *)rc, (void *)yc, (void *)tv,
                    (void *)info, (void *)Bt_inv, (void *)yt, (void *)fix_count, (void *)dinv32, (void *)bar,
                    (void *)Bt_raw, (void *)Bt_rawA, (void *)Ainv})
      if (q) (void)hipFree(q);
  }
};

inline int coarse_setup(Coarse &c, const std::vector<int32_t> &tile_start, const std::vector<int64_t> &tile_brick,
                        const BrickGrid &grid, const double *xyz_dev_order, int64_t N, int max_dofs,
                        const std::vector<int32_t> &conn, bool local = false, bool multi_rank = false, int modes = 6) {
  const int64_t T = (int64_t)tile_start.size() - 1;
  c.cm = modes;
  const int64_t *nbrick = grid.nb;
  int ax[3] = {0, 1, 2};
  std::stable_sort(ax, ax + 3, [&](int l, int r) { return nbrick[l] > nbrick[r]; });
  auto grid_agg = [&](int64_t key, int , const int64_t *na) {
    const int64_t b[3] = {key / (nbrick[2] * nbrick[1]), (key / nbrick[2]) % nbrick[1], key % nbrick[2]};
    const int64_t a0 = b[ax[0]] * na[ax[0]] / nbrick[ax[0]], a1 = b[ax[1]] * na[ax[1]] / nbrick[ax[1]],
                  a2 = b[ax[2]] * na[ax[2]] / nbrick[ax[2]];
    return (a0 * na[ax[1]] + a1) * na[ax[2]] + a2;
  };
  int g = 2;
  int64_t na[3];
  std::vector<int64_t> used;
  for (int step = 0;; ++step) {
    const double scale = 1.5 + 0.125 * step;
    for (int k = 0; k < 3; ++k) na[k] = std::max<int64_t>(1, (int64_t)std::floor((double)nbrick[k] / scale));
    if (!local && step == 0 && grid.na[0] > 0 && modes * grid.na[0] * grid.na[1] * grid.na[2] <= max_dofs)
      for (int k = 0; k < 3; ++k) na[k] = grid.na[k];
    int64_t count = na[0] * na[1] * na[2];
    if (local) {
      used.clear();
      for (int64_t t = 0; t < T; ++t) used.push_back(grid_agg(tile_brick[t], g, na));
      std::sort(used.begin(), used.end());
      used.erase(std::unique(used.begin(), used.end()), used.end());
      count = (int64_t)used.size();
    }
    if (count * modes <= max_dofs || scale > 64.0) break;
  }
  const int n_agg = local ? (int)used.size() : (int)(na[0] * na[1] * na[2]);
  std::vector<int32_t> agg_of_tile(T), agg_of_node(N);
  std::vector<double> cen((size_t)n_agg * 3, 0.0);
  for (int a = 0; a < n_agg; ++a) {
    const int64_t ga = local ? used[a] : a;
    int64_t ai[3];
    ai[ax[0]] = ga / (na[ax[1]] * na[ax[2]]);
    ai[ax[1]] = (ga / na[ax[2]]) % na[ax[1]];
    ai[ax[2]] = ga % na[ax[2]];
    for (int k = 0; k < 3; ++k) {
      const int64_t b_lo = (ai[k] * nbrick[k] + na[k] - 1) / na[k], b_hi = ((ai[k] + 1) * nbrick[k] + na[k] - 1) / na[k];
      cen[3 * a + k] = grid.lo[k] + 0.5 * (double)(b_lo + b_hi) * grid.side[k];
    }
  }
  for (int64_t t = 0; t < T; ++t) {
    const int64_t ga = grid_agg(tile_brick[t], g, na);
    const int a = local ? (int)(std::lower_bound(used.begin(), used.end(), ga) - used.begin()) : (int)ga;
    agg_of_tile[t] = a;
    for (int32_t i = tile_start[t]; i < tile_start[t + 1]; ++i) agg_of_node[i] = a;
  }
  {
    if (hipMalloc((void **)&c.dinv32, (size_t)N * 6 * sizeof(float)) != hipSuccess) return 2;
    c.rel_exact = false;
    if (!local && xyz_dev_order && !std::getenv("PL_NO_REL32")) {
      std::vector<float> rel((size_t)N * 3);
      bool exact = true;
      for (int64_t i = 0; i < N && exact; ++i)
        for (int k = 0; k < 3; ++k) {
          const double d = xyz_dev_order[3 * i + k] - cen[3 * (size_t)agg_of_node[i] + k];
          const float f = (float)d;
          if ((double)f != d) {
            exact = false;
            break;
          }
          rel[3 * (size_t)i + k] = f;
        }
      if (exact) {
        if (c.rel32.upload(rel) != hipSuccess) return 1;
        c.rel_exact = true;
      }
    }
  }
  c.n_agg = n_agg;
  c.nc = modes * n_agg;
  c.n_tiles = T;
  {
    int longest = 1;
    for (int64_t t = 0; t < T; ++t) longest = std::max(longest, (int)(tile_start[t + 1] - tile_start[t]));
    c.vblock = std::min(kBlock, (longest + kWave - 1) / kWave * kWave);
  }
  {
    const int64_t B = (int64_t)conn.size() / 2;
    std::vector<std::pair<int64_t, int32_t>> cross;
    std::vector<int32_t> tile_of_node(N);
    for (int64_t t = 0; t < T; ++t)
      for (int32_t i = tile_start[t]; i < tile_start[t + 1]; ++i) tile_of_node[i] = (int32_t)t;
    if (c.tile_of_node.upload(tile_of_node) != hipSuccess) return 1;
    for (int64_t b = 0; b < B; ++b) {
      const int I = agg_of_node[conn[2 * b]], J = agg_of_node[conn[2 * b + 1]];
      if (I != J || (modes == 12 && tile_of_node[conn[2 * b]] != tile_of_node[conn[2 * b + 1]]))
        cross.push_back({(int64_t)I * n_agg + J, (int32_t)b});
    }
    int64_t max_diff = std::min<int64_t>(n_agg - 1, na[ax[1]] * na[ax[2]] + na[ax[2]] + 1);
    if (local) {
      max_diff = 0;
      for (const auto &pr : cross) max_diff = std::max<int64_t>(max_diff, std::abs(pr.first / n_agg - pr.first % n_agg));
    }
    c.bw_blocks = (int)((modes * (max_diff + 1) + kNB - 1) / kNB + 1);
    for (const auto &pr : cross)
      if (std::abs(pr.first / n_agg - pr.first % n_agg) > max_diff) {
        if (multi_rank && !local) return 4;
        c.bw_blocks = 0;
      }
    std::sort(cross.begin(), cross.end());
    std::vector<int32_t> idx2;
    idx2.reserve(cross.size() + cross.size() / 2);
    for (size_t q = 0; q < cross.size(); ++q) {
      if (q > 0 && cross[q].first != cross[q - 1].first)
        while (idx2.size() % kWave) idx2.push_back(-1);
      idx2.push_back(cross[q].second);
    }
    while (idx2.size() % kWave) idx2.push_back(-1);
    c.n_cross = (int64_t)idx2.size();
    if (c.cross_idx.upload(idx2) != hipSuccess) return 1;
  }
  if (c.agg_of_node.upload(agg_of_node) != hipSuccess || c.agg_of_tile.upload(agg_of_tile) != hipSuccess ||
      c.cen.upload(cen) != hipSuccess)
    return 1;
  c.ncp = (c.nc + kNB - 1) / kNB * kNB;
  const size_t n2 = (size_t)c.ncp * c.ncp;
  if (hipMalloc((void **)&c.Ac, n2 * sizeof(double)) != hipSuccess) return 2;
  c.ac_clean = false;
  if (hipMalloc((void **)&c.W, n2 * sizeof(float)) != hipSuccess) return 2;
  if (hipMalloc((void **)&c.Lf, n2 * sizeof(double)) != hipSuccess) return 2;
  if (hipMemset(c.Lf, 0, n2 * sizeof(double)) != hipSuccess) return 2;
  if (hipMalloc((void **)&c.Wt, n2 * sizeof(float)) != hipSuccess) return 2;
  if (hipMalloc((void **)&c.Dinv, (size_t)c.ncp * kNB * sizeof(double)) != hipSuccess) return 2;
  if (hipMalloc((void **)&c.rc, (size_t)(c.ncp + 2 * kSlots) * sizeof(double)) != hipSuccess) return 2;
  if (hipMalloc((void **)&c.yc, (size_t)c.ncp * sizeof(double)) != hipSuccess) return 2;
  if (hipMalloc((void **)&c.tv, (size_t)c.ncp * sizeof(double)) != hipSuccess) return 2;
  if (hipMalloc((void **)&c.info, 2 * sizeof(int)) != hipSuccess) return 2;
  if (hipMalloc((void **)&c.bar, sizeof(unsigned)) != hipSuccess) return 2;
  {
    c.h_tile_start = tile_start;
    if (hipMalloc((void **)&c.Bt_inv, (size_t)T * 144 * sizeof(double)) != hipSuccess) return 2;
    if (hipMalloc((void **)&c.Bt_raw, (size_t)T * 144 * sizeof(double)) != hipSuccess) return 2;
    if (hipMalloc((void **)&c.yt, (size_t)T * 12 * sizeof(double)) != hipSuccess) return 2;
    if (hipMemset(c.Bt_inv, 0, (size_t)T * 144 * sizeof(double)) != hipSuccess) return 2;
    if (hipMemset(c.Bt_raw, 0, (size_t)T * 144 * sizeof(double)) != hipSuccess) return 2;
    if (hipMemset(c.yt, 0, (size_t)T * 12 * sizeof(double)) != hipSuccess) return 2;
  }
  if (hipMemset(c.rc, 0, (size_t)(c.ncp + 2 * kSlots) * sizeof(double)) != hipSuccess) return 2;
  if (hipMemset(c.W, 0, n2 * sizeof(float)) != hipSuccess) return 2;
  if (hipMemset(c.Wt, 0, n2 * sizeof(float)) != hipSuccess) return 2;
  c.enabled = true;
  return 0;
}

__global__ __launch_bounds__(kBlock) void k_list_fixed_struts(int64_t B, const int32_t *__restrict__ conn,
                                                              const int32_t *__restrict__ agg,
                                                              const uint8_t *__restrict__ fixedbits,
                                                              int64_t *__restrict__ keys, int *__restrict__ count) {
  const int64_t b = (int64_t)blockIdx.x * kBlock + threadIdx.x;
// ... 560 lines not shown
    for (int q = 0; q < kBlock / kWave; ++q) v += red[threadIdx.x][q];
    if (threadIdx.x < 21) {
      int q = 0;
      while ((q + 1) * (q + 2) / 2 <= (int)threadIdx.x) ++q;
      const int p = (int)threadIdx.x - q * (q + 1) / 2;
      B[(6 + p) * 12 + 6 + q] = v;
      B[(6 + q) * 12 + 6 + p] = v;
    } else {
      const int e = (int)threadIdx.x - 21, p = e / 6, q = e % 6;
      B[p * 12 + 6 + q] = v;
      B[(6 + q) * 12 + p] = v;
    }
  }
}
constexpr int kInv12Block = 192;
__global__ __launch_bounds__(kInv12Block) void k_tile_invert12(int64_t T, const double *__restrict__ raw,
                                                              double *__restrict__ Bt_inv) {
  constexpr int n = 12;
  __shared__ double A[n][n + 1];
  __shared__ double diag0[n];
  const int64_t t = blockIdx.x;
  if (t >= T) return;
  const int e = threadIdx.x, i = e / n, j = e - n * i;
  const bool act = e < n * n;
  if (act) A[i][j] = 0.5 * (raw[t * 144 + i * n + j] + raw[t * 144 + j * n + i]);
  __syncthreads();
  if (e < n) diag0[e] = A[e][e];
  __syncthreads();
  unsigned dropped = 0u;
  for (int k = 0; k < n; ++k) {
    const double d = A[k][k];
    if (!(d > 1e-10 * diag0[k]) || !(diag0[k] > 0.0)) {
      dropped |= 1u << k;
      continue;
    }
    const double inv = 1.0 / d;
    double v = 0.0;
    if (act) {
      const bool di = (dropped >> i) & 1u, dj = (dropped >> j) & 1u;
      if (i == k && j == k) v = -inv;
      else if (i == k) v = A[k][j] * inv;
      else if (j == k) v = A[k][i] * inv;
      else if (di || dj) v = A[i][j];
      else v = A[i][j] - (A[i][k] * inv) * A[k][j];
    }
    __syncthreads();
    if (act) A[i][j] = v;
    __syncthreads();
  }
  if (act) {
    const bool out = ((dropped >> i) & 1u) || ((dropped >> j) & 1u);
    Bt_inv[t * 144 + i * n + j] = out ? 0.0 : -A[i][j];
  }
}
inline void coarse_factor(Coarse &cs, int n, hipStream_t s, const std::function<void(int)> &after_chol, unsigned *bar,
                          TrtriPhases ph = TrtriPhases()) {
  if (cs.w16)
    dense_factor_inverse(cs.Ac, cs.Lf, reinterpret_cast<bf16_t *>(cs.W), reinterpret_cast<bf16_t *>(cs.Wt), cs.Dinv, n, n,
                         cs.info, cs.bw_blocks, s, after_chol, bar, ph);
  else
    dense_factor_inverse(cs.Ac, cs.Lf, cs.W, cs.Wt, cs.Dinv, n, n, cs.info, cs.bw_blocks, s, after_chol, bar, ph);
}
constexpr int kOneGemvMaxDofs = 2048;
inline void coarse_apply(const Coarse &cs, const double *r, double *t, double *y, double *dot_out, const double *add0,
                         hipStream_t s) {
  static const bool one_off = [] { const char *e = std::getenv("PL_ONE_GEMV"); return e && e[0] == '0'; }();
  if (cs.ainv_ready && cs.Ainv && cs.ncp <= kOneGemvMaxDofs && !one_off) {
    hipLaunchKernelGGL(k_full_gemv, dim3((cs.ncp + 3) / 4), dim3(kBlock), 0, s, cs.ncp, (const float *)cs.Ainv, cs.ncp, r, y,
                       dot_out, add0);
    return;
  }
  if (cs.w16)
    dense_apply(reinterpret_cast<const bf16_t *>(cs.W), reinterpret_cast<const bf16_t *>(cs.Wt), cs.ncp, cs.ncp, r, t, y,
                dot_out, add0, s);
  else
    dense_apply(cs.W, cs.Wt, cs.ncp, cs.ncp, r, t, y, dot_out, add0, s);
}

__global__ __launch_bounds__(kBlock) void k_to_float(int64_t n, const double *__restrict__ x, float *__restrict__ y) {
  const int64_t i = (int64_t)blockIdx.x * kBlock + threadIdx.x;
  if (i < n) y[i] = (float)x[i];
}

template <typename PT, typename RT, int TM = 6, bool MULTI = true, bool LOCAL = true>
__global__ __launch_bounds__(kBlock) void k_pcg_update_tile(const int32_t *__restrict__ tile_start,
                                                            const int32_t *__restrict__ agg_of_tile,
                                                            const double *__restrict__ cen,
                                                            const double *__restrict__ xyz,
                                                            const PT *__restrict__ Ap,
                                                            const float *__restrict__ dinv32,
                                                            const double *__restrict__ w ,
                                                            RT *__restrict__ r,
                                                            double *__restrict__ scal, double *__restrict__ rc,
                                                            const double *__restrict__ Bt_inv ,
                                                            double *__restrict__ yt,
                                                            const int32_t *__restrict__ aggL_of_tile ,
                                                            const double *__restrict__ cenL,
                                                            const uint8_t *__restrict__ shared ,
                                                            double *__restrict__ rcL, int ncp,
                                                            const uint8_t *__restrict__ skip_rows ,
                                                            int cm = 6 ,
                                                            const float *__restrict__ rel32 = nullptr ) {
  __shared__ double red[32][4 * kBlock / kWave];
  if constexpr (!MULTI) {
    w = nullptr;
    shared = nullptr;
  }
  if constexpr (!MULTI || !LOCAL) aggL_of_tile = nullptr;
  double *rr_slot = rc + ncp + (blockIdx.x & (kSlots - 1)), *rdr_slot = rr_slot + kSlots;
  const int t = blockIdx.x;
  double pap, old_rz;
  scalar_read2(scal, S_PAP, S_RZ_OLD, pap, old_rz);
  const double alpha = (pap != 0.0) ? old_rz / pap : 0.0;
  const int n0 = tile_start[t], n1 = tile_start[t + 1];
  const int a = agg_of_tile[t];
  const double c0 = cen[3 * a], c1 = cen[3 * a + 1], c2 = cen[3 * a + 2];
  __shared__ double sbi[16][TM];
  double bi[TM];
#pragma unroll
  for (int j = 0; j < TM; ++j) bi[j] = 0.0;
  const int my_mode = (TM == 12) ? ((int)threadIdx.x < 6 ? (int)threadIdx.x : ((int)threadIdx.x >= 8 && (int)threadIdx.x < 14
                                                                                   ? (int)threadIdx.x - 2 : -1))
                                 : ((int)threadIdx.x < 6 ? (int)threadIdx.x : -1);
  if (Bt_inv && my_mode >= 0) {
#pragma unroll
    for (int j = 0; j < TM; ++j) bi[j] = Bt_inv[(size_t)t * (TM * TM) + TM * my_mode + j];
  }
  if (threadIdx.x < 16) {
#pragma unroll
    for (int j = 0; j < TM; ++j) sbi[threadIdx.x][j] = bi[j];
  }
  double accS[6] = {0, 0, 0, 0, 0, 0};
  double accD[6] = {0, 0, 0, 0, 0, 0};
  double acc[8] = {0, 0, 0, 0, 0, 0, 0, 0};
  const int aL = aggL_of_tile ? aggL_of_tile[t] : 0;
  double l0 = 0.0, l1 = 0.0, l2 = 0.0;
  if (aggL_of_tile) {
    l0 = cenL[3 * aL];
    l1 = cenL[3 * aL + 1];
    l2 = cenL[3 * aL + 2];
  }
  double accL[6] = {0, 0, 0, 0, 0, 0};
  double accT[6] = {0, 0, 0, 0, 0, 0};
  const bool own_t = Bt_inv && shared;
  for (int i = n0 + threadIdx.x; i < n1; i += blockDim.x) {
    if (skip_rows && skip_rows[i]) continue;
    double av[6], dv[6], rv[6];
    const float2 *d2 = reinterpret_cast<const float2 *>(dinv32 + 6 * (int64_t)i);
#pragma unroll
    for (int k = 0; k < 3; ++k) {
      const double2 aa = load_pair(Ap, 3 * (int64_t)i + k), rr = load_pair(r, 3 * (int64_t)i + k);
      const float2 dd = d2[k];
      av[2 * k] = aa.x; av[2 * k + 1] = aa.y;
      dv[2 * k] = dd.x; dv[2 * k + 1] = dd.y;
      rv[2 * k] = rr.x; rv[2 * k + 1] = rr.y;
    }
#pragma unroll
    for (int k = 0; k < 6; ++k) rv[k] -= alpha * av[k];
#pragma unroll
    for (int k = 0; k < 3; ++k) store_pair(r, 3 * (int64_t)i + k, double2{rv[2 * k], rv[2 * k + 1]});
    if (sizeof(RT) == 4) {
#pragma unroll
      for (int k = 0; k < 6; ++k) rv[k] = (double)(float)rv[k];
    }
    double wt[6] = {1, 1, 1, 1, 1, 1};
    if (w) {
#pragma unroll
      for (int k = 0; k < 6; ++k) wt[k] = w[6 * (int64_t)i + k];
    }
    double rx, ry, rz;
    if (rel32) {
      rx = (double)rel32[3 * (int64_t)i];
      ry = (double)rel32[3 * (int64_t)i + 1];
      rz = (double)rel32[3 * (int64_t)i + 2];
    } else {
      rx = xyz[3 * (int64_t)i] - c0;
      ry = xyz[3 * (int64_t)i + 1] - c1;
      rz = xyz[3 * (int64_t)i + 2] - c2;
    }
    const double ru[3] = {wt[0] * rv[0], wt[1] * rv[1], wt[2] * rv[2]};
    acc[0] += ru[0];
    acc[1] += ru[1];
    acc[2] += ru[2];
    acc[3] += wt[3] * rv[3] + (ry * ru[2] - rz * ru[1]);
    acc[4] += wt[4] * rv[4] + (rz * ru[0] - rx * ru[2]);
    acc[5] += wt[5] * rv[5] + (rx * ru[1] - ry * ru[0]);
#pragma unroll
    for (int k = 0; k < 6; ++k) {
      acc[6] += wt[k] * rv[k] * rv[k];
      acc[7] += wt[k] * dv[k] * rv[k] * rv[k];
    }
    if (TM == 12 && cm == 12 && shared) {
      accD[0] += rx * ru[0];
      accD[1] += ry * ru[1];
      accD[2] += rz * ru[2];
      accD[3] += 0.5 * (ry * ru[0] + rx * ru[1]);
      accD[4] += 0.5 * (rz * ru[1] + ry * ru[2]);
      accD[5] += 0.5 * (rz * ru[0] + rx * ru[2]);
    }
    if (TM == 12 && !(shared && shared[i])) {
      accS[0] += rx * ru[0];
      accS[1] += ry * ru[1];
      accS[2] += rz * ru[2];
      accS[3] += 0.5 * (ry * ru[0] + rx * ru[1]);
      accS[4] += 0.5 * (rz * ru[1] + ry * ru[2]);
      accS[5] += 0.5 * (rz * ru[0] + rx * ru[2]);
    }
    if (own_t && !shared[i]) {
      accT[0] += rv[0];
      accT[1] += rv[1];
      accT[2] += rv[2];
      accT[3] += rv[3] + (ry * rv[2] - rz * rv[1]);
      accT[4] += rv[4] + (rz * rv[0] - rx * rv[2]);
      accT[5] += rv[5] + (rx * rv[1] - ry * rv[0]);
    }
    if (aggL_of_tile && !(shared && shared[i])) {
      const double sx = xyz[3 * (int64_t)i] - l0, sy = xyz[3 * (int64_t)i + 1] - l1, sz = xyz[3 * (int64_t)i + 2] - l2;
      accL[0] += rv[0];
      accL[1] += rv[1];
      accL[2] += rv[2];
      accL[3] += rv[3] + (sy * rv[2] - sz * rv[1]);
      accL[4] += rv[4] + (sz * rv[0] - sx * rv[2]);
      accL[5] += rv[5] + (sx * rv[1] - sy * rv[0]);
    }
  }
  const int lane = threadIdx.x & 63, wv = threadIdx.x >> 6;
  const int nw = 4 * (blockDim.x >> 6);
  const bool row_end = (lane & 15) == 15;
  const int slot = 4 * wv + (lane >> 4);
#pragma unroll
  for (int k = 0; k < 8; ++k) {
    const double s = row_sums(acc[k]);
    if (row_end) red[k][slot] = s;
  }
  if (aggL_of_tile) {
#pragma unroll
    for (int k = 0; k < 6; ++k) {
      const double s = row_sums(accL[k]);
      if (row_end) red[8 + k][slot] = s;
    }
  }
  if (own_t) {
#pragma unroll
    for (int k = 0; k < 6; ++k) {
      const double s = row_sums(accT[k]);
      if (row_end) red[14 + k][slot] = s;
    }
  }
  if (TM == 12) {
#pragma unroll
    for (int k = 0; k < 6; ++k) {
      const double s = row_sums(accS[k]);
      if (row_end) red[20 + k][slot] = s;
    }
// ... 124 lines not shown
                                                     const int64_t *__restrict__ slice_ptr,
                                                     const int2 *__restrict__ ent, const uint16_t *__restrict__ pal,
                                                     unsigned long long *__restrict__ key) {
  const int64_t q = (int64_t)blockIdx.x * kBlock + threadIdx.x;
  if (q >= nc) return;
  const int64_t i = cnodes[q], s = i / SN, lane = i % SN;
  const int64_t p0 = slice_ptr[s], width = (slice_ptr[s + 1] - p0) / SN;
  unsigned long long h = 0;
  for (int64_t j = 0; j < width; ++j) {
    const int2 e = ent[p0 + j * SN + lane];
    if (e.x < 0) continue;
    unsigned long long v = ((unsigned long long)pal[e.y & 0x7fffffff] << 1) | (e.y < 0 ? 1ull : 0ull);
    v = (v + 0x9E3779B97F4A7C15ull) * 0xBF58476D1CE4E5B9ull;
    v ^= v >> 29;
    v *= 0x94D049BB133111EBull;
    v ^= v >> 32;
    h += v;
  }
  key[q] = h == ~0ull ? 0 : h;
}
__device__ __forceinline__ int cls_probe(unsigned long long h, unsigned long long *__restrict__ keys,
                                         int *__restrict__ owner, int q) {
  unsigned slot = (unsigned)(h >> 48);
  for (int probe = 0; probe < 32; ++probe) {
    unsigned long long cur = __hip_atomic_load(keys + slot, __ATOMIC_RELAXED, __HIP_MEMORY_SCOPE_AGENT);
    if (cur == ~0ull) cur = atomicCAS(keys + slot, ~0ull, h);
    if (cur == ~0ull || cur == h) {
      if (q < __hip_atomic_load(owner + slot, __ATOMIC_RELAXED, __HIP_MEMORY_SCOPE_AGENT)) atomicMin(owner + slot, q);
      return (int)slot;
    }
    slot = (slot + 1) & 65535u;
  }
  return -1;
}
__global__ __launch_bounds__(kBlock) void k_cls_insert(int64_t nc, const unsigned long long *__restrict__ key,
                                                       unsigned long long *__restrict__ keys, int *__restrict__ owner,
                                                       uint16_t *__restrict__ cls, int *__restrict__ flags) {
  const int64_t q = (int64_t)blockIdx.x * kBlock + threadIdx.x;
  const bool valid = q < nc;
  const unsigned long long h = valid ? key[q] : 0ull;
  const int lane = threadIdx.x & 63;
  int found = -2;
  unsigned long long todo = __ballot(valid);
  for (int round = 0; round < 12 && todo; ++round) {
    const int leader = __ffsll((long long)todo) - 1;
    const unsigned long long hl =
        ((unsigned long long)(unsigned)__builtin_amdgcn_readlane((int)(h >> 32), leader) << 32) |
        (unsigned long long)(unsigned)__builtin_amdgcn_readlane((int)(h & 0xFFFFFFFFull), leader);
    const unsigned long long same = __ballot(valid && found == -2 && h == hl);
    int sl = 0;
    if (lane == leader) sl = cls_probe(h, keys, owner, (int)q);
    sl = __builtin_amdgcn_readlane(sl, leader);
    if ((same >> lane) & 1ull) found = sl;
    todo &= ~same;
  }
  if (valid && found == -2) found = cls_probe(h, keys, owner, (int)q);
  if (valid) {
    if (found < 0) flags[0] = 1;
    else cls[q] = (uint16_t)found;
  }
}
__global__ __launch_bounds__(kBlock) void k_cls_publish(int64_t nc, const double *__restrict__ inv,
                                                        const int *__restrict__ owner, const uint16_t *__restrict__ cls,
                                                        double *__restrict__ table) {
  const int64_t t = (int64_t)blockIdx.x * kBlock + threadIdx.x;
  const int64_t q = t / 36;
  if (q >= nc) return;
  if (owner[cls[q]] == (int)q) table[36 * (int64_t)cls[q] + (t - 36 * q)] = inv[t];
}
__global__ __launch_bounds__(kBlock) void k_cls_verify(int64_t nc, const double *__restrict__ inv,
                                                       const uint16_t *__restrict__ cls,
                                                       const double *__restrict__ table, int *__restrict__ flags) {
  const int64_t q = (int64_t)blockIdx.x * kBlock + threadIdx.x;
  if (q >= nc) return;
  const double *a = inv + 36 * q, *b = table + 36 * (int64_t)cls[q];
  double scale = 0.0, diff = 0.0;
#pragma unroll
  for (int e = 0; e < 36; ++e) {
    scale = fmax(scale, fabs(a[e]));
    diff = fmax(diff, fabs(a[e] - b[e]));
  }
  if (!(diff <= 1e-10 * scale)) flags[0] = 1;
}
template <typename VT>
__global__ __launch_bounds__(kBlock) void k_condense_subtract(int64_t N, const uint8_t *__restrict__ cflag,
                                                              const VT *__restrict__ y, VT *__restrict__ r) {
  const int64_t t = (int64_t)blockIdx.x * kBlock + threadIdx.x;
  if (t >= 6 * N) return;
  if (!cflag[t / 6]) r[t] = (VT)((double)r[t] - (double)y[t]);
}
template <typename VT>
__global__ __launch_bounds__(kBlock) void k_condense_backsubst(int64_t nc, const int32_t *__restrict__ cnodes,
                                                               const double *__restrict__ inv,
                                                               const uint16_t *__restrict__ cls,
                                                               const VT *__restrict__ b,
                                                               const VT *__restrict__ y, VT *__restrict__ x) {
  const int64_t t = (int64_t)blockIdx.x * kBlock + threadIdx.x;
  const int64_t q = t / 6;
  const int k = (int)(t - 6 * q);
  if (q >= nc) return;
  const int64_t i = cnodes[q];
  const double *A = inv + 36 * (cls ? (int64_t)cls[q] : q);
  double acc = 0.0;
#pragma unroll
  for (int j = 0; j < 6; ++j) acc += A[6 * k + j] * ((double)b[6 * i + j] - (double)y[6 * i + j]);
  x[6 * i + k] = (VT)acc;
}

template <typename PT, typename RT, int TM = 6, bool MULTI = true, bool LOCAL = true>
__global__ __launch_bounds__(kBlock) void k_pcg_direction_coarse(const int32_t *__restrict__ tile_start,
                                                                 const RT *__restrict__ r,
                                                                 const float *__restrict__ dinv32,
                                                                 const double *__restrict__ xyz,
                                                                 const int32_t *__restrict__ agg_of_tile,
                                                                 const double *__restrict__ cen,
                                                                 const double *__restrict__ yc,
                                                                 const double *__restrict__ yt ,
                                                                 const uint8_t *__restrict__ fixedbits,
                                                                 PT *__restrict__ p, RT *__restrict__ x,
                                                                 const double *__restrict__ scal,
                                                                 double *__restrict__ scal_next,
                                                                 double *__restrict__ hist, int k,
                                                                 double *__restrict__ rc, int ncp,
                                                                 const int32_t *__restrict__ aggL_of_tile ,
                                                                 const double *__restrict__ cenL,
                                                                 const double *__restrict__ ycL,
                                                                 const uint8_t *__restrict__ shared ,
                                                                 double *__restrict__ rcL, int ncpL,
                                                                 const uint8_t *__restrict__ zero_rows ,
                                                                 int cm = 6,
                                                                 const float *__restrict__ rel32 = nullptr ) {
  if constexpr (!MULTI) shared = nullptr;
  if constexpr (!MULTI || !LOCAL) aggL_of_tile = nullptr;
  double old, rz_new, pap;
  scalar_read3(scal, S_RZ_OLD, S_RZ_NEW, S_PAP, old, rz_new, pap);
  const double beta = (old != 0.0) ? rz_new / old : 0.0;
  const double alpha = (pap != 0.0) ? old / pap : 0.0;
  if (blockIdx.x == 1 || gridDim.x == 1)
    for (int e = threadIdx.x; e < ncp; e += blockDim.x) rc[e] = 0.0;
  if (aggL_of_tile && (blockIdx.x == 2 || gridDim.x <= 2))
    for (int e = threadIdx.x; e < ncpL; e += blockDim.x) rcL[e] = 0.0;
  if (blockIdx.x == 0 && threadIdx.x < kWave) {
    const int s = threadIdx.x;
    double rr = 0.0;
    for (int q = s; q < kSlots; q += kWave) rr += rc[ncp + q];
    rr = wave_sum(rr);
    if (s == 0) hist[k] = rr;
    for (int q = s; q < kSlots; q += kWave) {
      rc[ncp + q] = 0.0;
      rc[ncp + kSlots + q] = 0.0;
      scal_next[S_RZ_OLD * kSlots + q] = scal[S_RZ_NEW * kSlots + q];
      scal_next[S_RZ_NEW * kSlots + q] = 0.0;
      scal_next[S_PAP * kSlots + q] = 0.0;
    }
  }
  const int t = blockIdx.x;
  const int n0 = tile_start[t], n1 = tile_start[t + 1];
  const int a = agg_of_tile[t];
  const double *y = yc + cm * a;
  double U0 = y[0], U1 = y[1], U2 = y[2], W0 = y[3], W1 = y[4], W2 = y[5];
  double T[TM];
#pragma unroll
  for (int k = 0; k < TM; ++k) T[k] = 0.0;
  if (yt) {
    const double *q = yt + TM * (size_t)t;
#pragma unroll
    for (int k = 0; k < TM; ++k) T[k] = q[k];
    if (!shared) {
      U0 += T[0]; U1 += T[1]; U2 += T[2]; W0 += T[3]; W1 += T[4]; W2 += T[5];
    }
  }
  double ED[6] = {0, 0, 0, 0, 0, 0};
  if constexpr (TM == 12) {
    if (cm == 12) {
#pragma unroll
      for (int k = 0; k < 6; ++k) ED[k] = y[6 + k];
      if (!shared) {
#pragma unroll
        for (int k = 0; k < 6; ++k) {
          T[6 + k] += ED[k];
          ED[k] = 0.0;
        }
      }
    }
  }
  const bool own_t = yt && shared;
  const double c0 = cen[3 * a], c1 = cen[3 * a + 1], c2 = cen[3 * a + 2];
  double L[6] = {0, 0, 0, 0, 0, 0}, l0 = 0.0, l1 = 0.0, l2 = 0.0;
  if (aggL_of_tile) {
    const int aL = aggL_of_tile[t];
#pragma unroll
    for (int q = 0; q < 6; ++q) L[q] = ycL[6 * aL + q];
    l0 = cenL[3 * aL];
    l1 = cenL[3 * aL + 1];
    l2 = cenL[3 * aL + 2];
  }
  for (int64_t i = n0 + threadIdx.x; i < n1; i += blockDim.x) {
    if (zero_rows && zero_rows[i]) continue;
    double rx, ry, rz;
    if (rel32) {
      rx = (double)rel32[3 * i];
      ry = (double)rel32[3 * i + 1];
      rz = (double)rel32[3 * i + 2];
    } else {
      rx = xyz[3 * i] - c0;
      ry = xyz[3 * i + 1] - c1;
      rz = xyz[3 * i + 2] - c2;
    }
    double zc[6] = {U0 + (W1 * rz - W2 * ry), U1 + (W2 * rx - W0 * rz), U2 + (W0 * ry - W1 * rx), W0, W1, W2};
    if constexpr (TM == 12) {
     if (shared && cm == 12) {
      zc[0] += ED[0] * rx + 0.5 * (ED[3] * ry + ED[5] * rz);
      zc[1] += ED[1] * ry + 0.5 * (ED[3] * rx + ED[4] * rz);
      zc[2] += ED[2] * rz + 0.5 * (ED[4] * ry + ED[5] * rx);
     }
     if (!(shared && shared[i])) {
      zc[0] += T[6] * rx + 0.5 * (T[9] * ry + T[11] * rz);
      zc[1] += T[7] * ry + 0.5 * (T[9] * rx + T[10] * rz);
      zc[2] += T[8] * rz + 0.5 * (T[10] * ry + T[11] * rx);
     }
    }
    if (own_t && !shared[i]) {
      zc[0] += T[0] + (T[4] * rz - T[5] * ry);
      zc[1] += T[1] + (T[5] * rx - T[3] * rz);
      zc[2] += T[2] + (T[3] * ry - T[4] * rx);
      zc[3] += T[3];
      zc[4] += T[4];
      zc[5] += T[5];
    }
    if (aggL_of_tile && !(shared && shared[i])) {
      const double sx = xyz[3 * i] - l0, sy = xyz[3 * i + 1] - l1, sz = xyz[3 * i + 2] - l2;
      zc[0] += L[0] + (L[4] * sz - L[5] * sy);
      zc[1] += L[1] + (L[5] * sx - L[3] * sz);
      zc[2] += L[2] + (L[3] * sy - L[4] * sx);
      zc[3] += L[3];
      zc[4] += L[4];
      zc[5] += L[5];
    }
    const unsigned fb = fixedbits[i];
    const float2 *d2 = reinterpret_cast<const float2 *>(dinv32 + 6 * i);
#pragma unroll
    for (int q = 0; q < 3; ++q) {
      const double2 rr = load_pair(r, 3 * i + q);
      const float2 dd = d2[q];
      double2 pp = load_pair(p, 3 * i + q);
      double2 xx = load_pair(x, 3 * i + q);
      xx.x += alpha * pp.x;
      xx.y += alpha * pp.y;
      store_pair(x, 3 * i + q, xx);
      const double z0 = dd.x * rr.x + (((fb >> (2 * q)) & 1u) ? 0.0 : zc[2 * q]);
      const double z1 = dd.y * rr.y + (((fb >> (2 * q + 1)) & 1u) ? 0.0 : zc[2 * q + 1]);
      pp.x = z0 + beta * pp.x;
      pp.y = z1 + beta * pp.y;
      store_pair(p, 3 * i + q, pp);
    }
  }
}

template <typename PT, typename RT, int TM>
__global__ __launch_bounds__(kBlock) void k_pcg_direction_flat(int64_t N, const int32_t *__restrict__ tile_of_node,
                                                               const RT *__restrict__ r,
                                                               const float *__restrict__ dinv32,
                                                               const double *__restrict__ xyz,
                                                               const int32_t *__restrict__ agg_of_tile,
                                                               const double *__restrict__ cen,
                                                               const double *__restrict__ yc,
                                                               const double *__restrict__ yt ,
                                                               const uint8_t *__restrict__ fixedbits,
                                                               PT *__restrict__ p, RT *__restrict__ x,
                                                               const double *__restrict__ scal,
                                                               double *__restrict__ scal_next,
                                                               double *__restrict__ hist, int k,
                                                               double *__restrict__ rc, int ncp,
                                                               const int32_t *__restrict__ keep ,
                                                               int cm, const uint8_t *__restrict__ shared ,
                                                               const float *__restrict__ rel32 = nullptr ) {
  double old, rz_new, pap;
  scalar_read3(scal, S_RZ_OLD, S_RZ_NEW, S_PAP, old, rz_new, pap);
  const double beta = (old != 0.0) ? rz_new / old : 0.0;
  const double alpha = (pap != 0.0) ? old / pap : 0.0;
  if (blockIdx.x == 1 || gridDim.x == 1)
    for (int e = threadIdx.x; e < ncp; e += blockDim.x) rc[e] = 0.0;
  if (blockIdx.x == 0 && threadIdx.x < kWave) {
    const int s = threadIdx.x;
    double rr = 0.0;
    for (int q = s; q < kSlots; q += kWave) rr += rc[ncp + q];
    rr = wave_sum(rr);
    if (s == 0) hist[k] = rr;
    for (int q = s; q < kSlots; q += kWave) {
      rc[ncp + q] = 0.0;
      rc[ncp + kSlots + q] = 0.0;
      scal_next[S_RZ_OLD * kSlots + q] = scal[S_RZ_NEW * kSlots + q];
      scal_next[S_RZ_NEW * kSlots + q] = 0.0;
      scal_next[S_PAP * kSlots + q] = 0.0;
    }
  }
  const int64_t lane_pair = (int64_t)blockIdx.x * blockDim.x + threadIdx.x;
  if (lane_pair >= 3 * N) return;
  const int64_t slot = lane_pair / 3;
  const int q = (int)(lane_pair - 3 * slot);
  const int64_t i = keep ? (int64_t)keep[slot] : slot;
  const int64_t pair = 3 * i + q;
  const int t = tile_of_node[i];
  const int a = agg_of_tile[t];
  const double *y = yc + cm * a;
  double C[12];
#pragma unroll
  for (int m = 0; m < 6; ++m) C[m] = y[m];
#pragma unroll
  for (int m = 6; m < 12; ++m) C[m] = 0.0;
  if constexpr (TM == 12) {
    if (cm == 12) {
#pragma unroll
      for (int m = 6; m < 12; ++m) C[m] = y[m];
    }
  }
  if (yt && !(shared && shared[i])) {
    const double *w = yt + TM * (size_t)t;
#pragma unroll
    for (int m = 0; m < TM; ++m) C[m] += w[m];
  }
  double rx, ry, rz;
  if (rel32) {
    rx = (double)rel32[3 * i];
    ry = (double)rel32[3 * i + 1];
    rz = (double)rel32[3 * i + 2];
  } else {
    rx = xyz[3 * i] - cen[3 * a];
    ry = xyz[3 * i + 1] - cen[3 * a + 1];
    rz = xyz[3 * i + 2] - cen[3 * a + 2];
  }
  double zc[6] = {C[0] + (C[4] * rz - C[5] * ry), C[1] + (C[5] * rx - C[3] * rz), C[2] + (C[3] * ry - C[4] * rx),
                  C[3], C[4], C[5]};
  if constexpr (TM == 12) {
    zc[0] += C[6] * rx + 0.5 * (C[9] * ry + C[11] * rz);
    zc[1] += C[7] * ry + 0.5 * (C[9] * rx + C[10] * rz);
    zc[2] += C[8] * rz + 0.5 * (C[10] * ry + C[11] * rx);
  }
  double z0 = q == 0 ? zc[0] : (q == 1 ? zc[2] : zc[4]);
  double z1 = q == 0 ? zc[1] : (q == 1 ? zc[3] : zc[5]);
  const unsigned fb = fixedbits[i];
  const float2 dd = reinterpret_cast<const float2 *>(dinv32)[pair];
  const double2 rr = load_pair(r, pair);
  double2 pp = load_pair(p, pair);
  double2 xx = load_pair(x, pair);
  xx.x += alpha * pp.x;
  xx.y += alpha * pp.y;
  store_pair(x, pair, xx);
  z0 = dd.x * rr.x + (((fb >> (2 * q)) & 1u) ? 0.0 : z0);
  z1 = dd.y * rr.y + (((fb >> (2 * q + 1)) & 1u) ? 0.0 : z1);
  pp.x = z0 + beta * pp.x;
  pp.y = z1 + beta * pp.y;
  store_pair(p, pair, pp);
}

}
```

### pylatticedso_amd/csrc/pl_context.h

```cpp
#pragma once
#include <hip/hip_runtime.h>

#include <algorithm>
#include <atomic>
#include <chrono>
#include <cmath>
#include <cstdlib>
#include <cstdio>
#include <cstring>
#include <functional>
#include <memory>
#include <numeric>
#include <string>
#include <vector>

#include "../../include/pylattice_hip.h"
#include "pl_kernels.h"
#include "pl_parallel.h"
#include "pl_tile.h"
#include "pl_rows.h"
#include "pl_dist.h"
#include "pl_coarse.h"
#include "pl_cg1.h"
#include "pl_small.h"
// ... 88 lines not shown
  DevBuf<double> xprev;
  bool xprev_valid = false;
  int pal_fail_streak = 0, pal_skip_left = 0;
  bool pal_skipped = false;
  DevBuf<double> xprev2;
  bool xprev2_valid = false;
  DevBuf<double> xprev3;
  bool xprev3_valid = false;
  static constexpr int kWarmMax = 8;
  DevBuf<double> gh[kWarmMax - 1];
  int gh_head = 0, gh_count = 0;
  DevBuf<double> gw[kWarmMax];
  DevBuf<double> gw_dots;
  DevBuf<double> cg1;
  int hist_cap = 0;
  pl::TilePlan tile;
  int opkind = 0;
  int64_t ddm_cells = 0;
  int ddm_nb = 0;
  int ddm_n_S = 0;
  std::vector<int32_t> h_ddm_cell_nodes, h_ddm_cell_S;
  DevBuf<int32_t> ddm_cell_nodes, ddm_cell_S;
  DevBuf<double> ddm_St;
  DevBuf<double> ddm_Sraw;
  DevBuf<int64_t> ddm_node_ptr;
  DevBuf<int32_t> ddm_node_ent;
  DevBuf<double> ddm_stage;
  DevBuf<int32_t> ddm_order;
  DevBuf<int32_t> ddm_tiles, ddm_tile_S;
  int64_t ddm_n_tiles = 0;
  DevBuf<int32_t> ddm_tile_gidx;
  DevBuf<int32_t> ddm_cell_P;
  DevBuf<double> ddm_Pt;
  bool ddm_have_P = false;
  DevBuf<double> dd_A, dd_Lf, dd_W, dd_Wt, dd_Dinv, dd_tv;
  DevBuf<int> dd_info;
  int dd_n = 0;
  int dd_bw = 0;
  bool dd_ready = false;
  DevBuf<double> dd_B;
  bool dd_blocks = false;
  DevBuf<double> dd2_xyz, dd2_cen;
  DevBuf<int32_t> dd2_agg, dd2_ptr, dd2_nodes;
  pl::Coarse dd2;
  int dd2_n_agg = 0;
  bool dd2_plan = false, dd2_ready = false;
  DevBuf<int> stop_flag;
  bool stop_use = false;
  double stop_thresh = 0.0;
  DevBuf<unsigned long long> pal_keys;
  DevBuf<int> pal_owner, pal_flags;
  DevBuf<uint16_t> pal_id;
  DevBuf<int> pal_dense_of_slot;
  DevBuf<pl::Record> pal_dense;
  DevBuf<uint32_t> vword;
  DevBuf<uint32_t> vword_dir;
  bool vword_dir_fresh = false;
  bool pal_lds = false;
  pl::RowPlan rows;
  DevBuf<uint32_t> rword;
  DevBuf<pl::Record> pal_dense2;
  bool pal_rows = false;
  DevBuf<pl::Record> palette;
  bool pal_ready = false;
  int pal_entries = 0;
  pl::Coarse coarse;
  int coarse_info = 0;
  pl::Coarse coarseL;
  DevBuf<uint8_t> sharedbits, maskL;
  std::vector<uint8_t> h_cand;
  std::vector<uint8_t> h_shared;
  DevBuf<uint8_t> cend;
  DevBuf<int32_t> cnodes, cbase;
  DevBuf<int32_t> ckeep;
  int cbase_state = -1;
  DevBuf<double> kcc_inv;
  DevBuf<uint8_t> maskC, cflag;
  DevBuf<unsigned long long> cls_key, cls_keys;
  DevBuf<int> cls_owner, cls_flags;
  DevBuf<uint16_t> cls_id;
  DevBuf<double> cls_table;
  int *cls_host_flag = nullptr;
  bool cls_ready = false;
  DevBuf<double> p2, small_scal, small_rc;
  bool small_use = false;
  bool persist_use = false;
  DevBuf<double> ps_Ug, ps_red;
  DevBuf<unsigned> ps_flags;
  DevBuf<unsigned long long> ps_dbg;
  DevBuf<int32_t> ps_agg_ptr, ps_agg_idx;
  int ps_n_agg = 0;
  int last_iterations = 0;
  int64_t n_cond = 0;
  bool cond_ready = false;
  bool cond_use = false;
  int cond_agree = -1;
  pl::Dist dist;
  std::vector<int32_t> h_tile_start;
  DevBuf<int32_t> ov_iface, ov_inner;
  int64_t n_ov_iface = 0, n_ov_inner = 0;
  bool ov_ready = false;
  hipStream_t comm_stream = nullptr;
  hipEvent_t ev_ov_a = nullptr, ev_ov_x = nullptr;

  pl_stats_t last{};
  double ms_assembly = 0.0;
  double *pin6 = nullptr;
  size_t pin6_n = 0;
  DevBuf<int32_t> per_ptr, per_nodes;
  int64_t n_per_groups = 0;
  double *pinB = nullptr;
  DevBuf<double> sens_out;
  DevBuf<double> usol;
  bool usol_valid = false;
  std::shared_ptr<void> multi_ws;
  std::shared_ptr<void> geom_ws;
  DevBuf<double> st_vm4, st_part, st_red, st_G, st_dr;

  ~pl_context() {
    if (ev0) (void)hipEventDestroy(ev0);
    if (ev1) (void)hipEventDestroy(ev1);
    if (ev_fork) (void)hipEventDestroy(ev_fork);
    if (ev_join) (void)hipEventDestroy(ev_join);
    if (ev_chol) (void)hipEventDestroy(ev_chol);
    if (ev_fill1) (void)hipEventDestroy(ev_fill1);
    if (ev_p0) (void)hipEventDestroy(ev_p0);
    if (ev_p1) (void)hipEventDestroy(ev_p1);
    if (ev_t0) (void)hipEventDestroy(ev_t0);
    if (ev_t1) (void)hipEventDestroy(ev_t1);
    if (pin6) (void)hipHostFree(pin6);
    if (pinB) (void)hipHostFree(pinB);
    if (ev_ov_a) (void)hipEventDestroy(ev_ov_a);
    if (ev_ov_x) (void)hipEventDestroy(ev_ov_x);
    if (comm_stream) (void)hipStreamDestroy(comm_stream);
    if (side2) (void)hipStreamDestroy(side2);
    if (side_cu) (void)hipStreamDestroy(side_cu);
    if (side) (void)hipStreamDestroy(side);
    if (stream) (void)hipStreamDestroy(stream);
  }
};

namespace {

int staging(pl_context *c, double **out) {
  const size_t n6 = (size_t)c->N * 6;
  if (!c->pin6 || c->pin6_n < n6) {
    if (c->pin6) (void)hipHostFree(c->pin6);
    c->pin6 = nullptr;
    void *p = nullptr;
    PL_HIP(hipHostMalloc(&p, n6 * sizeof(double), hipHostMallocDefault));
    c->pin6 = static_cast<double *>(p);
    c->pin6_n = n6;
  }
  *out = c->pin6;
  return PL_OK;
}

int stagingB(pl_context *c, double **out) {
  if (!c->pinB) {
    void *p = nullptr;
    PL_HIP(hipHostMalloc(&p, (size_t)std::max<int64_t>(c->B, 1) * sizeof(double), hipHostMallocDefault));
    c->pinB = static_cast<double *>(p);
  }
  *out = c->pinB;
  return PL_OK;
}
// ... 39 lines not shown
```

### pylatticedso_amd/csrc/pl_solver.h

```cpp
#pragma once
#include "pl_assembly.h"

namespace {

__global__ __launch_bounds__(pl::kBlock) void k_warm_mask(int64_t N, const uint8_t *__restrict__ cflag ,
                                                         const uint8_t *__restrict__ fixed, double *__restrict__ p) {
  const int64_t t = (int64_t)blockIdx.x * pl::kBlock + threadIdx.x;
  if (t < 6 * N && ((cflag && cflag[t / 6]) || fixed[t])) p[t] = 0.0;
}
__global__ __launch_bounds__(pl::kBlock) void k_warm_extrapolate(int64_t n6, const double *__restrict__ a ,
                                                                 const double *__restrict__ b , double *__restrict__ p) {
  const int64_t t = (int64_t)blockIdx.x * pl::kBlock + threadIdx.x;
  if (t < n6) p[t] = 2.0 * a[t] - b[t];
}
__global__ __launch_bounds__(pl::kBlock) void k_warm_extrapolate2(int64_t n6, const double *__restrict__ a, const double *__restrict__ b,
                                                                  const double *__restrict__ c3, double *__restrict__ p) {
  const int64_t t = (int64_t)blockIdx.x * pl::kBlock + threadIdx.x;
  if (t < n6) p[t] = 3.0 * (a[t] - b[t]) + c3[t];
}
constexpr int kWarmMax = pl_context::kWarmMax;
struct WarmVecs {
  const double *v[kWarmMax];
};
struct WarmCoef {
  double c[kWarmMax];
};
__global__ __launch_bounds__(pl::kBlock) void k_warm_dots(int64_t N, int m, WarmVecs V, int j, const uint8_t *__restrict__ cflag,
                                                          const double *__restrict__ Ap, const double *__restrict__ r,
                                                          double *__restrict__ out ) {
  __shared__ double red[kWarmMax + 1][pl::kBlock / pl::kWave];
  double acc[kWarmMax + 1];
#pragma unroll
  for (int i = 0; i <= kWarmMax; ++i) acc[i] = 0.0;
  for (int64_t t = (int64_t)blockIdx.x * pl::kBlock + threadIdx.x; t < 6 * N; t += (int64_t)gridDim.x * pl::kBlock) {
    if (cflag && cflag[t / 6]) continue;
    const double a = Ap[t];
#pragma unroll
    for (int i = 0; i < kWarmMax; ++i)
      if (i < m) acc[i] += V.v[i][t] * a;
    acc[kWarmMax] += V.v[j][t] * r[t];
  }
  const int lane = threadIdx.x & 63, wv = threadIdx.x >> 6;
#pragma unroll
  for (int i = 0; i <= kWarmMax; ++i) {
    const double s = pl::wave_sum(acc[i]);
    if (lane == 0) red[i][wv] = s;
  }
  __syncthreads();
  if (threadIdx.x <= kWarmMax) {
    double s = 0.0;
    for (int w = 0; w < pl::kBlock / pl::kWave; ++w) s += red[threadIdx.x][w];
    const int i = threadIdx.x;
    if (i < m) unsafeAtomicAdd(out + i, s);
    else if (i == kWarmMax) unsafeAtomicAdd(out + m, s);
  }
}
__global__ __launch_bounds__(pl::kBlock) void k_warm_combine(int64_t n6, int m, WarmVecs V, WarmCoef C, double *__restrict__ p) {
  const int64_t t = (int64_t)blockIdx.x * pl::kBlock + threadIdx.x;
  if (t >= n6) return;
  double s = 0.0;
#pragma unroll
  for (int i = 0; i < kWarmMax; ++i)
    if (i < m) s += C.c[i] * V.v[i][t];
  p[t] = s;
}
__global__ __launch_bounds__(pl::kBlock) void k_warm_apply(int64_t N, const uint8_t *__restrict__ cflag ,
                                                          const double *__restrict__ Ap, const double *__restrict__ p,
                                                          double *__restrict__ r, double *__restrict__ x) {
  const int64_t t = (int64_t)blockIdx.x * pl::kBlock + threadIdx.x;
  if (t >= 6 * N) return;
  if (cflag && cflag[t / 6]) return;
  r[t] -= Ap[t];
  x[t] = p[t];
}

template <typename PT, typename RT>
int pcg_tail_coarse_t(pl_context *c, double *cur, double *nxt, int hist_slot, PT *p, const PT *Ap, RT *x, RT *r) {
  pl::Coarse &cs = c->coarse, &cl = c->coarseL;
  const bool useL = cl.ready;
#define PL_UPD(TM, MULTI, LOCAL)                                                                                    \
  hipLaunchKernelGGL((pl::k_pcg_update_tile<PT, RT, TM, MULTI, LOCAL>), dim3((unsigned)cs.n_tiles), dim3(cs.vblock), \
                     0, c->stream,                                                                                   \
                     c->tile.tile_start.p, cs.agg_of_tile.p, cs.cen.p, c->xyz.p, Ap, cs.dinv32,                       \
                     c->dist.active ? (const double *)c->dist.weight.p : (const double *)nullptr, r, cur,             \
                     cs.rc, cs.tile_level ? (const double *)cs.Bt_inv : (const double *)nullptr, cs.yt,               \
                     useL ? (const int32_t *)cl.agg_of_tile.p : (const int32_t *)nullptr, cl.cen.p,                   \
                     (c->dist.active || useL) ? (const uint8_t *)c->sharedbits.p : (const uint8_t *)nullptr, cl.rc,   \
                     cs.ncp, c->cond_use ? (const uint8_t *)c->cflag.p : (const uint8_t *)nullptr, cs.cm, rel32)
  const float *rel32 = cs.rel_exact ? (const float *)cs.rel32.p : (const float *)nullptr;
  if (useL) {
    if (tile_modes_now(c) == 12) PL_UPD(12, true, true);
    else PL_UPD(6, true, true);
  } else if (c->dist.active) {
    if (tile_modes_now(c) == 12) PL_UPD(12, true, false);
    else PL_UPD(6, true, false);
  } else if (tile_modes_now(c) == 12) PL_UPD(12, false, false);
  else PL_UPD(6, false, false);
#undef PL_UPD
  if (useL)
    pl::coarse_apply(cl, cl.rc, cl.tv, cl.yc, cs.rc + cs.ncp + pl::kSlots, (const double *)nullptr, c->stream);
  if (c->dist.active) {
    if (pl::dist_sum_scalars(c->dist, cs.rc, cs.ncp + 2 * pl::kSlots, c->stream))
      return fail(PL_ERR_HIP, "RCCL all-reduce of the coarse residual failed");
  }
  pl::coarse_apply(cs, cs.rc, cs.tv, cs.yc, cur + pl::S_RZ_NEW * pl::kSlots, cs.rc + cs.ncp + pl::kSlots, c->stream);
#define PL_DIR(TM, MULTI, LOCAL)                                                                                         \
  hipLaunchKernelGGL((pl::k_pcg_direction_coarse<PT, RT, TM, MULTI, LOCAL>), dim3((unsigned)cs.n_tiles), dim3(cs.vblock), \
                     0, c->stream,                                                                                        \
                     c->tile.tile_start.p, (const RT *)r, cs.dinv32, c->xyz.p, cs.agg_of_tile.p, cs.cen.p, cs.yc,         \
                     cs.tile_level ? (const double *)cs.yt : (const double *)nullptr, c->fixedbits.p, p, x, cur, nxt,     \
                     c->hist.p, hist_slot, cs.rc, cs.ncp,                                                                \
                     useL ? (const int32_t *)cl.agg_of_tile.p : (const int32_t *)nullptr, cl.cen.p, cl.yc,                \
                     (c->dist.active || useL) ? (const uint8_t *)c->sharedbits.p : (const uint8_t *)nullptr, cl.rc,       \
                     cl.ncp, c->cond_use ? (const uint8_t *)c->cflag.p : (const uint8_t *)nullptr, cs.cm, rel32)
  const int64_t n_flat = c->cond_use ? c->N - c->n_cond : c->N;
#define PL_DIRF(TM)                                                                                                      \
  hipLaunchKernelGGL((pl::k_pcg_direction_flat<PT, RT, TM>), dim3((unsigned)((3 * n_flat + pl::kBlock - 1) / pl::kBlock)), \
                     dim3(pl::kBlock), 0, c->stream, n_flat, cs.tile_of_node.p, (const RT *)r, cs.dinv32, c->xyz.p,       \
                     cs.agg_of_tile.p, cs.cen.p, cs.yc, cs.tile_level ? (const double *)cs.yt : (const double *)nullptr,  \
                     c->fixedbits.p, p, x, cur, nxt, c->hist.p, hist_slot, cs.rc, cs.ncp,                                \
                     c->cond_use ? (const int32_t *)c->ckeep.p : (const int32_t *)nullptr, cs.cm,                        \
                     c->dist.active ? (const uint8_t *)c->sharedbits.p : (const uint8_t *)nullptr, rel32)
  if (!useL && sizeof(PT) == 8) {
    if (tile_modes_now(c) == 12) PL_DIRF(12);
    else PL_DIRF(6);
  } else if (useL) {
    if (tile_modes_now(c) == 12) PL_DIR(12, true, true);
    else PL_DIR(6, true, true);
  } else if (c->dist.active) {
    if (tile_modes_now(c) == 12) PL_DIR(12, true, false);
    else PL_DIR(6, true, false);
  } else if (tile_modes_now(c) == 12) PL_DIR(12, false, false);
  else PL_DIR(6, false, false);
#undef PL_DIRF
#undef PL_DIR
  PL_HIP(hipGetLastError());
  return PL_OK;
}

int pcg_tail_coarse(pl_context *c, double *cur, double *nxt, int hist_slot) {
  return pcg_tail_coarse_t<double, double>(c, cur, nxt, hist_slot, c->p.p, (const double *)c->Ap.p, c->x.p, c->r.p);
}

inline void ddm_precondition(pl_context *c, double *dot, bool restricted = false) {
  if (c->dd2_ready) {
    pl::Coarse &cs = c->dd2;
    const uint8_t *fx = c->have_bc ? (const uint8_t *)c->fixed.p : (const uint8_t *)nullptr;
    if (!restricted)
      hipLaunchKernelGGL(pl::k_ddm_restrict, dim3((unsigned)c->dd2_n_agg), dim3(pl::kBlock), 0, c->stream, c->dd2_ptr.p,
                         c->dd2_nodes.p, (const double *)c->dd2_cen.p, (const double *)c->dd2_xyz.p, fx,
                         (const double *)c->r.p, cs.rc);
    pl::coarse_apply(cs, cs.rc, cs.tv, cs.yc, dot, (const double *)nullptr, c->stream);
    hipLaunchKernelGGL(pl::k_ddm_two_level_apply, dim3(grid_for(c->N * 6)), dim3(pl::kBlock), 0, c->stream, c->N,
                       (const double *)c->dd_B.p, c->dd2_agg.p, (const double *)c->dd2_cen.p, (const double *)c->dd2_xyz.p, fx,
                       (const double *)cs.yc, (const double *)c->r.p, c->z.p, dot, cs.rc, cs.ncp);
    return;
  }
  if (c->dd_ready)
    pl::dense_apply(c->dd_W.p, c->dd_Wt.p, c->dd_n, c->dd_n, c->r.p, c->dd_tv.p, c->z.p, dot, (const double *)nullptr,
                    c->stream);
  else
    hipLaunchKernelGGL(pl::k_ddm_node_blocks_apply, dim3(grid_for(c->N * 6)), dim3(pl::kBlock), 0, c->stream, c->N,
                       (const double *)c->dd_B.p, (const double *)c->r.p, c->z.p, dot);
}

inline int small_set_size() { return pl::S_COUNT * pl::kSlots; }
inline double *small_set(pl_context *c, int k) { return c->small_scal.p + (size_t)((k + 4) & 3) * small_set_size(); }
inline double *small_rc(pl_context *c, int parity) { return c->small_rc.p + (size_t)(parity & 1) * (c->coarse.ncp + 2 * pl::kSlots); }

int small_prepare(pl_context *c) {
  const int64_t n6 = c->N * 6;
  const size_t nrc = 2 * (size_t)(c->coarse.ncp + 2 * pl::kSlots);
  if (!c->p2.p || c->p2.n < (size_t)n6) PL_HIP(c->p2.alloc((size_t)n6));
  if (!c->small_scal.p) PL_HIP(c->small_scal.alloc(4 * (size_t)small_set_size()));
  if (!c->small_rc.p || c->small_rc.n < nrc) PL_HIP(c->small_rc.alloc(nrc));
  PL_HIP(hipMemsetAsync(c->small_scal.p, 0, 4 * (size_t)small_set_size() * sizeof(double), c->stream));
  PL_HIP(hipMemsetAsync(c->small_rc.p, 0, nrc * sizeof(double), c->stream));
  PL_HIP(hipMemsetAsync(c->p.p, 0, n6 * sizeof(double), c->stream));
  PL_HIP(hipMemsetAsync(c->p2.p, 0, n6 * sizeof(double), c->stream));
  return PL_OK;
}

int small_tail(pl_context *c, int k, int hist_slot) {
  pl::Coarse &cs = c->coarse;
  const uint8_t *skip = c->cond_use ? (const uint8_t *)c->cflag.p : (const uint8_t *)nullptr;
  const double *Bt = cs.tile_level ? (const double *)cs.Bt_inv : (const double *)nullptr;
  double *rc_new = small_rc(c, k + 1), *rc_old = small_rc(c, k);
#define PL_SUPD(TM)                                                                                                         \
  hipLaunchKernelGGL((pl::k_pcg_update_tile<double, double, TM, false, false>), dim3((unsigned)cs.n_tiles), dim3(cs.vblock),  \
                     0, c->stream, c->tile.tile_start.p, cs.agg_of_tile.p, cs.cen.p, c->xyz.p, (const double *)c->Ap.p,     \
                     cs.dinv32, (const double *)nullptr, c->r.p, small_set(c, k), rc_new, Bt, cs.yt,                        \
                     (const int32_t *)nullptr, (const double *)nullptr, (const uint8_t *)nullptr, (double *)nullptr, cs.ncp, \
                     skip, cs.cm)
#define PL_SZ(TM)                                                                                                           \
  hipLaunchKernelGGL((pl::k_small_z<TM>), dim3((unsigned)cs.n_tiles), dim3(cs.vblock), 0, c->stream, c->tile.tile_start.p,  \
                     cs.agg_of_tile.p, cs.cen.p, c->xyz.p, (const double *)c->r.p, cs.dinv32, c->fixedbits.p, skip,         \
                     (const float *)cs.Ainv, cs.ncp, cs.cm, (const double *)rc_new, rc_old,                                 \
                     cs.tile_level ? (const double *)cs.yt : (const double *)nullptr, c->z.p, small_set(c, k + 1),          \
                     small_set(c, k + 2), c->hist.p, hist_slot)
  if (tile_modes_now(c) == 12) {
    PL_SUPD(12);
    PL_SZ(12);
  } else {
    PL_SUPD(6);
    PL_SZ(6);
// ... 914 lines not shown
```

Baseline: 248.3 million.

## Compress per-node PCG data into packed words with deduplicated diagonal-inverse classes

Each node's offset from its aggregate centre is packed into a 32-bit word as three signed bytes with a shared power-of-two scale, used only when the packing is exact. Per-node float diagonal-inverse rows plus fixed bits are deduplicated into a table of at most 256 classes using a GPU hash table, and the class index goes in the word's top byte. The PCG update and direction kernels then read one word per node instead of separate rel32, dinv32 and fixedbits arrays, cutting memory traffic in the bandwidth-bound iteration. The cost is extra hashing, publish and verify kernels at assembly with a host readback, plus exponential backoff when classification fails; it is on by default unless PL_NODE_WORDS=0.

```diff
diff --git a/include/pylattice_hip.h b/include/pylattice_hip.h
--- a/include/pylattice_hip.h
+++ b/include/pylattice_hip.h
@@ -196,6 +196,7 @@
 
 int pl_time_kernel(pl_handle h, int which, int reps, double *avg_ms);
 int pl_algorithmic_bytes(pl_handle h, double *out3);
+int pl_node_words_info(pl_handle h, int *classes_on, int *n_classes, int *bytes_on, int *byte_exp);
 int pl_forget_history(pl_handle h);
 
 int pl_debug_spd_solve(int device, int32_t n, const double *A, const double *b, double *x, double *quad,
diff --git a/pylatticedso_amd/_capi.py b/pylatticedso_amd/_capi.py
--- a/pylatticedso_amd/_capi.py
+++ b/pylatticedso_amd/_capi.py
@@ -18,7 +18,7 @@
            "pl_spmv_free", "pl_spmv_bsr", "pl_solve", "pl_reactions", "pl_sens", "pl_energy", "pl_node_mod", "pl_schur",
            "pl_stress", "pl_stress_pnorm", "pl_buckling", "pl_buckling_pnorm",
            "pl_spmv_multi", "pl_solve_multi", "pl_schur_block", "pl_geom_spmv_multi", "pl_buckling_modes",
-           "pl_schur_cells", "pl_cells_recover", "pl_get_records", "pl_debug_partition", "pl_time_kernel", "pl_algorithmic_bytes", "pl_forget_history", "pl_debug_spd_solve", "pl_dist_unique_id_bytes",
+           "pl_schur_cells", "pl_cells_recover", "pl_get_records", "pl_debug_partition", "pl_time_kernel", "pl_algorithmic_bytes", "pl_node_words_info", "pl_forget_history", "pl_debug_spd_solve", "pl_dist_unique_id_bytes",
            "pl_dist_unique_id", "pl_dist_loopback_id", "pl_dist_abort", "pl_dist_init", "pl_dist_set_peers", "pl_generate_lattice", "pl_lattice_fetch",
            "pl_lattice_free", "pl_penalize", "pl_boundary_index", "pl_boundary_index_rows"]
 
@@ -94,7 +94,7 @@
            "pl_schur_cells": [V, I32, I32, I32, V, I32, V, V, V, V, V, V, V],
            "pl_cells_recover": [V, I32, I32, I32, V, I32, V, V, V, V, V, V, V, V, V, V, V],
            "pl_get_records": [V, V], "pl_debug_partition": [V, V, V, V, V], "pl_time_kernel": [V, I32, I32, V],
-           "pl_algorithmic_bytes": [V, V], "pl_forget_history": [V], "pl_debug_spd_solve": [I32, I32, V, V, V, V, I32], "pl_dist_unique_id_bytes": [], "pl_dist_unique_id": [V], "pl_dist_loopback_id": [V], "pl_dist_abort": [V],
+           "pl_algorithmic_bytes": [V, V], "pl_node_words_info": [V, V, V, V, V], "pl_forget_history": [V], "pl_debug_spd_solve": [I32, I32, V, V, V, V, I32], "pl_dist_unique_id_bytes": [], "pl_dist_unique_id": [V], "pl_dist_loopback_id": [V], "pl_dist_abort": [V],
            "pl_dist_init": [V, I32, I32, V, V, V, I32, I32], "pl_dist_set_peers": [V, V],
            "pl_generate_lattice": [I64, V, V, V, I32, I32, V, V, V, V], "pl_lattice_fetch": [V] * 12,
            "pl_lattice_free": [V], "pl_penalize": [I64, V, V, V, D, V, V, V],
@@ -701,6 +701,11 @@
         _check(self._lib, self._lib.pl_time_kernel(self._h, int(which), int(reps), C.byref(ms)))
         return ms.value
 
+    def node_words_info(self):
+        v = [C.c_int() for _ in range(4)]
+        _check(self._lib, self._lib.pl_node_words_info(self._h, *[C.byref(x) for x in v]))
+        return {"classes": bool(v[0].value), "n_classes": v[1].value, "bytes": bool(v[2].value), "byte_exp": v[3].value}
+
     def algorithmic_bytes(self):
         out = (C.c_double * 3)()
         _check(self._lib, self._lib.pl_algorithmic_bytes(self._h, out))
diff --git a/pylatticedso_amd/csrc/pl_api.hip b/pylatticedso_amd/csrc/pl_api.hip
--- a/pylatticedso_amd/csrc/pl_api.hip
+++ b/pylatticedso_amd/csrc/pl_api.hip
@@ -862,6 +862,7 @@
   pl::dist_destroy(h->dist);
   if (h->pal_host_flags != h->pal_fallback_flags) (void)hipHostFree(h->pal_host_flags);
   if (h->cls_host_flag) (void)hipHostFree(h->cls_host_flag);
+  if (h->dcl_host_flags) (void)hipHostFree(h->dcl_host_flags);
   delete h;
 }
 
@@ -904,6 +905,7 @@
   h->have_bc = true;
   h->coarse.n_fix = -1;
   h->coarseL.n_fix = -1;
+  h->coarse.dcl_ready = false;
   {
     int rcs = select_condensed(h, bits);
     if (rcs) return rcs;
@@ -931,11 +933,14 @@
     if (rc) return rc;
     rc = launch_dinv32(h);
     if (rc) return rc;
+    rc = launch_node_classes(h, h->stream, false);
+    if (rc) return rc;
     rc = agree_condensed(h);
     if (rc) return rc;
     rc = launch_condensed_blocks(h, h->stream);
     if (rc) return rc;
     PL_HIP(hipStreamSynchronize(h->stream));
+    finish_node_classes(h);
     {
       const bool keep = h->pal_ready;
       finish_condensed_classes(h);
@@ -1004,6 +1009,7 @@
   PL_HIP(hipMemcpyAsync(h->radius.p, stg, h->B * sizeof(double), hipMemcpyHostToDevice, h->stream));
   PL_HIP(hipStreamSynchronize(h->stream));
   h->assembled = false;
+  h->coarse.dcl_ready = false;
   h->have_bsr = false;
   return PL_OK;
 }
@@ -1023,6 +1029,7 @@
     PL_HIP(hipMemcpy(h->mult.p, m.data(), h->B * sizeof(double), hipMemcpyHostToDevice));
   }
   h->assembled = false;
+  h->coarse.dcl_ready = false;
   h->have_bsr = false;
   return PL_OK;
 }
@@ -1040,6 +1047,7 @@
   PL_HIP(hipMemcpy(h->seg_len.p, sl.data(), 3 * h->B * sizeof(double), hipMemcpyHostToDevice));
   PL_HIP(hipMemcpy(h->seg_nsub.p, sn.data(), 3 * h->B * sizeof(int32_t), hipMemcpyHostToDevice));
   h->assembled = false;
+  h->coarse.dcl_ready = false;
   h->have_bsr = false;
   return PL_OK;
 }
@@ -1202,17 +1210,32 @@
     rc = fem_factor_dense(h);
     if (rc) return rc;
   }
-  rc = build_coarse(h, h->coarse.enabled && h->have_bc ? std::function<void(int)>(queue_fill) : std::function<void(int)>());
+  bool dcl_queued = false;
+  int rc_dcl = PL_OK;
+  auto beside_chain = [&](int phase) {
+    if (!dcl_queued) {
+      dcl_queued = true;
+      rc_dcl = launch_node_classes(h, h->side, true);
+      if (!rc_dcl && hipEventRecord(h->ev_join, h->side) != hipSuccess)
+        rc_dcl = fail(PL_ERR_HIP, "pl_assemble: event record failed");
+    }
+    queue_fill(phase);
+  };
+  rc = build_coarse(h, h->coarse.enabled && h->have_bc ? std::function<void(int)>(beside_chain) : std::function<void(int)>());
   if (rc) return rc;
+  if (rc_dcl) return rc_dcl;
   queue_fill(1);
   if (rc_fill) return rc_fill;
   PL_HIP(hipStreamWaitEvent(h->stream, h->ev_join, 0));
-  rc = launch_dinv32(h);
-  if (rc) return rc;
+  if (!h->dcl_pending) {
+    rc = launch_dinv32(h);
+    if (rc) return rc;
+  }
   PL_HIP(hipEventRecord(h->ev1, h->stream));
   PL_HIP(hipStreamSynchronize(h->stream));
   finish_palette(h);
   finish_condensed_classes(h);
+  finish_node_classes(h);
   for (pl::Coarse *cs : {&h->coarse, &h->coarseL})
     if (cs->ready && cs->Ac) {
       PL_HIP(hipMemsetAsync(cs->Ac, 0, (size_t)cs->ncp * cs->ncp * sizeof(double), h->stream));
@@ -2435,6 +2458,19 @@
   return PL_OK;
 }
 
+int pl_node_words_info(pl_handle h, int *classes_on, int *n_classes, int *bytes_on, int *byte_exp) {
+  if (!valid(h)) return fail(PL_ERR_ARG, "pl_node_words_info: null handle");
+  const pl::Coarse &cs = h->coarse;
+  const bool words = node_words_apply(h);
+  const bool cls = words && h->assembled && cs.dcl_ready;
+  const bool bytes = words && cs.rel_e >= 0;
+  if (classes_on) *classes_on = cls ? 1 : 0;
+  if (n_classes) *n_classes = h->assembled ? cs.dcl_classes : 0;
+  if (bytes_on) *bytes_on = bytes ? 1 : 0;
+  if (byte_exp) *byte_exp = bytes ? cs.rel_e : -1;
+  return PL_OK;
+}
+
 int pl_debug_spd_solve(int device, int32_t n, const double *A, const double *b, double *x, double *quad,
                        int32_t fp32_factor) {
   return fp32_factor ? debug_spd_solve_t<float>(device, n, A, b, x, quad)
diff --git a/pylatticedso_amd/csrc/pl_assembly.h b/pylatticedso_amd/csrc/pl_assembly.h
--- a/pylatticedso_amd/csrc/pl_assembly.h
+++ b/pylatticedso_amd/csrc/pl_assembly.h
@@ -160,6 +160,66 @@
                      c->coarse.dinv32);
   PL_HIP(hipGetLastError());
   return PL_OK;
+}
+
+inline bool node_words_apply(const pl_context *c) {
+  return c->coarse.enabled && c->coarse.nword.p && !c->dist.active && !c->coarseL.ready;
+}
+int launch_node_classes(pl_context *c, hipStream_t st, bool convert) {
+  pl::Coarse &cs = c->coarse;
+  cs.dcl_ready = false;
+  cs.dcl_classes = 0;
+  c->dcl_pending = false;
+  if (!cs.enabled || !cs.nword.p || !cs.dcl_table || !c->have_bc || c->dist.active || c->coarseL.enabled)
+    return PL_OK;
+  if (c->dcl_skip_left > 0) {
+    c->dcl_skip_left--;
+    return PL_OK;
+  }
+  if (!c->dcl_keys.p) {
+    PL_HIP(c->dcl_keys.alloc(pl::kDclSlots));
+    PL_HIP(c->dcl_owner.alloc(pl::kDclSlots));
+    PL_HIP(c->dcl_dense_of_slot.alloc(pl::kDclSlots));
+    PL_HIP(c->dcl_flags.alloc(2));
+    PL_HIP(c->dcl_slot.alloc((size_t)c->N));
+    void *pinned = nullptr;
+    PL_HIP(hipHostMalloc(&pinned, 2 * sizeof(int), hipHostMallocDefault));
+    c->dcl_host_flags = static_cast<int *>(pinned);
+  }
+  c->dcl_host_flags[0] = 1;
+  c->dcl_host_flags[1] = 0;
+  PL_HIP(hipMemsetAsync(c->dcl_keys.p, 0xFF, pl::kDclSlots * sizeof(unsigned long long), st));
+  PL_HIP(hipMemsetAsync(c->dcl_owner.p, 0x7F, pl::kDclSlots * sizeof(int), st));
+  PL_HIP(hipMemsetAsync(c->dcl_dense_of_slot.p, 0xFF, pl::kDclSlots * sizeof(int), st));
+  PL_HIP(hipMemsetAsync(c->dcl_flags.p, 0, 2 * sizeof(int), st));
+  const dim3 g(grid_for(c->N)), blk(pl::kBlock);
+  if (convert)
+    hipLaunchKernelGGL(pl::k_to_float, dim3(grid_for(c->N * 6)), blk, 0, st, c->N * 6, c->dinv.p, cs.dinv32);
+  hipLaunchKernelGGL(pl::k_dcl_insert, g, blk, 0, st, c->N, (const float *)cs.dinv32, (const uint8_t *)c->fixedbits.p,
+                     c->dcl_keys.p, c->dcl_owner.p, c->dcl_slot.p, c->dcl_flags.p);
+  hipLaunchKernelGGL(pl::k_dcl_publish, g, blk, 0, st, c->N, (const float *)cs.dinv32, (const uint8_t *)c->fixedbits.p,
+                     (const int *)c->dcl_owner.p, (const uint16_t *)c->dcl_slot.p, c->dcl_dense_of_slot.p, cs.dcl_table,
+                     c->dcl_flags.p);
+  hipLaunchKernelGGL(pl::k_dcl_verify, g, blk, 0, st, c->N, (const float *)cs.dinv32, (const uint8_t *)c->fixedbits.p,
+                     (const uint16_t *)c->dcl_slot.p, (const int *)c->dcl_dense_of_slot.p, (const uint32_t *)cs.dcl_table,
+                     cs.nword.p, c->dcl_flags.p);
+  PL_HIP(hipGetLastError());
+  PL_HIP(hipMemcpyAsync(c->dcl_host_flags, c->dcl_flags.p, 2 * sizeof(int), hipMemcpyDeviceToHost, st));
+  c->dcl_pending = true;
+  return PL_OK;
+}
+void finish_node_classes(pl_context *c) {
+  if (!c->dcl_pending) return;
+  c->dcl_pending = false;
+  pl::Coarse &cs = c->coarse;
+  cs.dcl_classes = c->dcl_host_flags[1];
+  cs.dcl_ready = c->dcl_host_flags[0] == 0 && cs.dcl_classes > 0 && cs.dcl_classes <= pl::kDclMax;
+  if (cs.dcl_ready) {
+    c->dcl_fail_streak = 0;
+  } else {
+    c->dcl_fail_streak = std::min(c->dcl_fail_streak + 1, 4);
+    c->dcl_skip_left = (1 << c->dcl_fail_streak) - 1;
+  }
 }
 
 int launch_local_mask(pl_context *c) {
diff --git a/pylatticedso_amd/csrc/pl_coarse.h b/pylatticedso_amd/csrc/pl_coarse.h
--- a/pylatticedso_amd/csrc/pl_coarse.h
+++ b/pylatticedso_amd/csrc/pl_coarse.h
@@ -3,14 +3,22 @@
 
 #include <algorithm>
 #include <cstdint>
+#include <cstdlib>
 #include <vector>
 
 #include "pl_dense.h"
 #include "pl_kernels.h"
+#include "pl_nodeword.h"
 #include "pl_tile.h"
 
 namespace pl {
 
+constexpr int kDclMax = 256;
+constexpr int kDclSlots = 4096;
+inline bool node_words_enabled() {
+  const char *e = std::getenv("PL_NODE_WORDS");
+  return !(e && e[0] == '0');
+}
 
 struct Coarse {
   bool enabled = false;
@@ -42,13 +50,18 @@
   float *dinv32 = nullptr;
   TBuf<float> rel32;
   bool rel_exact = false;
+  TBuf<uint32_t> nword;
+  int rel_e = -1;
+  bool dcl_ready = false;
+  int dcl_classes = 0;
+  uint32_t *dcl_table = nullptr;
   TBuf<int32_t> fix_list;
   int *fix_count = nullptr;
   int64_t n_fix = -1;
   ~Coarse() {
     for (void *q : {(void *)Ac, (void *)Lf, (void *)W, (void *)Wt, (void *)Dinv, (void *)rc, (void *)yc, (void *)tv,
                     (void *)info, (void *)Bt_inv, (void *)yt, (void *)fix_count, (void *)dinv32, (void *)bar,
-                    (void *)Bt_raw, (void *)Bt_rawA, (void *)Ainv})
+                    (void *)Bt_raw, (void *)Bt_rawA, (void *)Ainv, (void *)dcl_table})
       if (q) (void)hipFree(q);
   }
 };
@@ -125,6 +138,18 @@
         if (c.rel32.upload(rel) != hipSuccess) return 1;
         c.rel_exact = true;
       }
+    }
+    c.rel_e = -1;
+    if (!local && xyz_dev_order && node_words_enabled()) {
+      std::vector<double> d((size_t)N * 3);
+      for (int64_t i = 0; i < N; ++i)
+        for (int k = 0; k < 3; ++k) d[3 * (size_t)i + k] = xyz_dev_order[3 * i + k] - cen[3 * (size_t)agg_of_node[i] + k];
+      std::vector<uint32_t> words;
+      int e = -1;
+      if (pack_rel_bytes(d.data(), (size_t)N, words, e)) c.rel_e = e;
+      else words.assign((size_t)N, 0u);
+      if (c.nword.upload(words) != hipSuccess) return 1;
+      if (hipMalloc((void **)&c.dcl_table, (size_t)kDclMax * 8 * sizeof(uint32_t)) != hipSuccess) return 2;
     }
   }
   c.n_agg = n_agg;
@@ -851,6 +876,12 @@
   if (i < n) y[i] = (float)x[i];
 }
 
+__device__ __forceinline__ void nword_rel(uint32_t w, double rscale, double &rx, double &ry, double &rz) {
+  rx = (double)((int)(w << 24) >> 24) * rscale;
+  ry = (double)((int)(w << 16) >> 24) * rscale;
+  rz = (double)((int)(w << 8) >> 24) * rscale;
+}
+
 template <typename PT, typename RT, int TM = 6, bool MULTI = true, bool LOCAL = true>
 __global__ __launch_bounds__(kBlock) void k_pcg_update_tile(const int32_t *__restrict__ tile_start,
                                                             const int32_t *__restrict__ agg_of_tile,
@@ -869,7 +900,10 @@
                                                             double *__restrict__ rcL, int ncp,
                                                             const uint8_t *__restrict__ skip_rows ,
                                                             int cm = 6 ,
-                                                            const float *__restrict__ rel32 = nullptr ) {
+                                                            const float *__restrict__ rel32 = nullptr ,
+                                                            const uint32_t *__restrict__ nword = nullptr ,
+                                                            const uint32_t *__restrict__ dtab = nullptr ,
+                                                            double rscale = 0.0 ) {
   __shared__ double red[32][4 * kBlock / kWave];
   if constexpr (!MULTI) {
     w = nullptr;
@@ -915,7 +949,9 @@
   for (int i = n0 + threadIdx.x; i < n1; i += blockDim.x) {
     if (skip_rows && skip_rows[i]) continue;
     double av[6], dv[6], rv[6];
-    const float2 *d2 = reinterpret_cast<const float2 *>(dinv32 + 6 * (int64_t)i);
+    const uint32_t nw = nword ? nword[i] : 0u;
+    const float2 *d2 = dtab ? reinterpret_cast<const float2 *>(dtab + 8 * (nw >> 24))
+                            : reinterpret_cast<const float2 *>(dinv32 + 6 * (int64_t)i);
 #pragma unroll
     for (int k = 0; k < 3; ++k) {
       const double2 aa = load_pair(Ap, 3 * (int64_t)i + k), rr = load_pair(r, 3 * (int64_t)i + k);
@@ -938,7 +974,9 @@
       for (int k = 0; k < 6; ++k) wt[k] = w[6 * (int64_t)i + k];
     }
     double rx, ry, rz;
-    if (rel32) {
+    if (rscale != 0.0) {
+      nword_rel(nw, rscale, rx, ry, rz);
+    } else if (rel32) {
       rx = (double)rel32[3 * (int64_t)i];
       ry = (double)rel32[3 * (int64_t)i + 1];
       rz = (double)rel32[3 * (int64_t)i + 2];
@@ -1229,6 +1267,113 @@
   }
   if (!(diff <= 1e-10 * scale)) flags[0] = 1;
 }
+__device__ __forceinline__ void dcl_row(const float *__restrict__ dinv32, const uint8_t *__restrict__ fixedbits, int64_t i,
+                                        uint32_t v[7]) {
+#pragma unroll
+  for (int k = 0; k < 6; ++k) v[k] = __float_as_uint(dinv32[6 * i + k]);
+  v[6] = fixedbits[i];
+}
+__device__ __forceinline__ unsigned long long dcl_hash(const uint32_t v[7]) {
+  unsigned long long h = 0x9E3779B97F4A7C15ull;
+#pragma unroll
+  for (int k = 0; k < 7; ++k) {
+    h = (h ^ v[k]) * 0xBF58476D1CE4E5B9ull;
+    h ^= h >> 29;
+  }
+  h *= 0x94D049BB133111EBull;
+  h ^= h >> 32;
+  return h == ~0ull ? 0 : h;
+}
+__device__ __forceinline__ int dcl_probe(unsigned long long h, unsigned long long *__restrict__ keys,
+                                         int *__restrict__ owner, int i) {
+  unsigned slot = (unsigned)(h >> 52) & (unsigned)(kDclSlots - 1);
+  for (int probe = 0; probe < 32; ++probe) {
+    unsigned long long cur = __hip_atomic_load(keys + slot, __ATOMIC_RELAXED, __HIP_MEMORY_SCOPE_AGENT);
+    if (cur == ~0ull) cur = atomicCAS(keys + slot, ~0ull, h);
+    if (cur == ~0ull || cur == h) {
+      if (i < __hip_atomic_load(owner + slot, __ATOMIC_RELAXED, __HIP_MEMORY_SCOPE_AGENT)) atomicMin(owner + slot, i);
+      return (int)slot;
+    }
+    slot = (slot + 1) & (unsigned)(kDclSlots - 1);
+  }
+  return -1;
+}
+__global__ __launch_bounds__(kBlock) void k_dcl_insert(int64_t N, const float *__restrict__ dinv,
+                                                       const uint8_t *__restrict__ fixedbits,
+                                                       unsigned long long *__restrict__ keys, int *__restrict__ owner,
+                                                       uint16_t *__restrict__ slot_of_node, int *__restrict__ flags) {
+  const int64_t i = (int64_t)blockIdx.x * kBlock + threadIdx.x;
+  const bool valid = i < N;
+  uint32_t v[7] = {0, 0, 0, 0, 0, 0, 0};
+  if (valid) dcl_row(dinv, fixedbits, i, v);
+  const unsigned long long h = valid ? dcl_hash(v) : 0ull;
+  const int lane = threadIdx.x & 63;
+  int found = -2;
+  unsigned long long todo = __ballot(valid);
+  for (int round = 0; round < 12 && todo; ++round) {
+    const int leader = __ffsll((long long)todo) - 1;
+    const unsigned long long hl =
+        ((unsigned long long)(unsigned)__builtin_amdgcn_readlane((int)(h >> 32), leader) << 32) |
+        (unsigned long long)(unsigned)__builtin_amdgcn_readlane((int)(h & 0xFFFFFFFFull), leader);
+    const unsigned long long same = __ballot(valid && found == -2 && h == hl);
+    int sl = 0;
+    if (lane == leader) sl = dcl_probe(h, keys, owner, (int)i);
+    sl = __builtin_amdgcn_readlane(sl, leader);
+    if ((same >> lane) & 1ull) found = sl;
+    todo &= ~same;
+  }
+  if (valid && found == -2) found = dcl_probe(h, keys, owner, (int)i);
+  if (valid) {
+    if (found < 0) flags[0] = 1;
+    slot_of_node[i] = (uint16_t)(found < 0 ? 0 : found);
+  }
+}
+__global__ __launch_bounds__(kBlock) void k_dcl_publish(int64_t N, const float *__restrict__ dinv,
+                                                        const uint8_t *__restrict__ fixedbits,
+                                                        const int *__restrict__ owner,
+                                                        const uint16_t *__restrict__ slot_of_node,
+                                                        int *__restrict__ dense_of_slot, uint32_t *__restrict__ table,
+                                                        int *__restrict__ flags) {
+  const int64_t i = (int64_t)blockIdx.x * kBlock + threadIdx.x;
+  if (i >= N) return;
+  const int slot = slot_of_node[i];
+  if (owner[slot] != (int)i) return;
+  const int d = atomicAdd(flags + 1, 1);
+  if (d >= kDclMax) {
+    flags[0] = 1;
+    return;
+  }
+  uint32_t v[7];
+  dcl_row(dinv, fixedbits, i, v);
+#pragma unroll
+  for (int k = 0; k < 7; ++k) table[8 * d + k] = v[k];
+  table[8 * d + 7] = 0u;
+  dense_of_slot[slot] = d;
+}
+__global__ __launch_bounds__(kBlock) void k_dcl_verify(int64_t N, const float *__restrict__ dinv,
+                                                       const uint8_t *__restrict__ fixedbits,
+                                                       const uint16_t *__restrict__ slot_of_node,
+                                                       const int *__restrict__ dense_of_slot,
+                                                       const uint32_t *__restrict__ table, uint32_t *__restrict__ nword,
+                                                       int *__restrict__ flags) {
+  const int64_t i = (int64_t)blockIdx.x * kBlock + threadIdx.x;
+  if (i >= N) return;
+  const int d = dense_of_slot[slot_of_node[i]];
+  if (d < 0 || d >= kDclMax) {
+    flags[0] = 1;
+    return;
+  }
+  uint32_t v[7];
+  dcl_row(dinv, fixedbits, i, v);
+  bool same = true;
+#pragma unroll
+  for (int k = 0; k < 7; ++k) same = same && table[8 * d + k] == v[k];
+  if (!same) {
+    flags[0] = 1;
+    return;
+  }
+  nword[i] = (nword[i] & 0x00FFFFFFu) | ((uint32_t)d << 24);
+}
 template <typename VT>
 __global__ __launch_bounds__(kBlock) void k_condense_subtract(int64_t N, const uint8_t *__restrict__ cflag,
                                                               const VT *__restrict__ y, VT *__restrict__ r) {
@@ -1276,7 +1421,10 @@
                                                                  double *__restrict__ rcL, int ncpL,
                                                                  const uint8_t *__restrict__ zero_rows ,
                                                                  int cm = 6,
-                                                                 const float *__restrict__ rel32 = nullptr ) {
+                                                                 const float *__restrict__ rel32 = nullptr ,
+                                                                 const uint32_t *__restrict__ nword = nullptr,
+                                                                 const uint32_t *__restrict__ dtab = nullptr,
+                                                                 double rscale = 0.0 ) {
   if constexpr (!MULTI) shared = nullptr;
   if constexpr (!MULTI || !LOCAL) aggL_of_tile = nullptr;
   double old, rz_new, pap;
@@ -1344,8 +1492,11 @@
   }
   for (int64_t i = n0 + threadIdx.x; i < n1; i += blockDim.x) {
     if (zero_rows && zero_rows[i]) continue;
+    const uint32_t nw = nword ? nword[i] : 0u;
     double rx, ry, rz;
-    if (rel32) {
+    if (rscale != 0.0) {
+      nword_rel(nw, rscale, rx, ry, rz);
+    } else if (rel32) {
       rx = (double)rel32[3 * i];
       ry = (double)rel32[3 * i + 1];
       rz = (double)rel32[3 * i + 2];
@@ -1384,8 +1535,9 @@
       zc[4] += L[4];
       zc[5] += L[5];
     }
-    const unsigned fb = fixedbits[i];
-    const float2 *d2 = reinterpret_cast<const float2 *>(dinv32 + 6 * i);
+    const uint32_t *row = dtab ? dtab + 8 * (nw >> 24) : nullptr;
+    const unsigned fb = dtab ? row[6] : (unsigned)fixedbits[i];
+    const float2 *d2 = dtab ? reinterpret_cast<const float2 *>(row) : reinterpret_cast<const float2 *>(dinv32 + 6 * i);
 #pragma unroll
     for (int q = 0; q < 3; ++q) {
       const double2 rr = load_pair(r, 3 * i + q);
@@ -1421,7 +1573,10 @@
                                                                double *__restrict__ rc, int ncp,
                                                                const int32_t *__restrict__ keep ,
                                                                int cm, const uint8_t *__restrict__ shared ,
-                                                               const float *__restrict__ rel32 = nullptr ) {
+                                                               const float *__restrict__ rel32 = nullptr ,
+                                                               const uint32_t *__restrict__ nword = nullptr,
+                                                               const uint32_t *__restrict__ dtab = nullptr,
+                                                               double rscale = 0.0 ) {
   double old, rz_new, pap;
   scalar_read3(scal, S_RZ_OLD, S_RZ_NEW, S_PAP, old, rz_new, pap);
   const double beta = (old != 0.0) ? rz_new / old : 0.0;
@@ -1467,8 +1622,11 @@
 #pragma unroll
     for (int m = 0; m < TM; ++m) C[m] += w[m];
   }
+  const uint32_t nw = nword ? nword[i] : 0u;
   double rx, ry, rz;
-  if (rel32) {
+  if (rscale != 0.0) {
+    nword_rel(nw, rscale, rx, ry, rz);
+  } else if (rel32) {
     rx = (double)rel32[3 * i];
     ry = (double)rel32[3 * i + 1];
     rz = (double)rel32[3 * i + 2];
@@ -1486,8 +1644,9 @@
   }
   double z0 = q == 0 ? zc[0] : (q == 1 ? zc[2] : zc[4]);
   double z1 = q == 0 ? zc[1] : (q == 1 ? zc[3] : zc[5]);
-  const unsigned fb = fixedbits[i];
-  const float2 dd = reinterpret_cast<const float2 *>(dinv32)[pair];
+  const uint32_t *row = dtab ? dtab + 8 * (nw >> 24) : nullptr;
+  const unsigned fb = dtab ? row[6] : (unsigned)fixedbits[i];
+  const float2 dd = dtab ? reinterpret_cast<const float2 *>(row)[q] : reinterpret_cast<const float2 *>(dinv32)[pair];
   const double2 rr = load_pair(r, pair);
   double2 pp = load_pair(p, pair);
   double2 xx = load_pair(x, pair);
diff --git a/pylatticedso_amd/csrc/pl_context.h b/pylatticedso_amd/csrc/pl_context.h
--- a/pylatticedso_amd/csrc/pl_context.h
+++ b/pylatticedso_amd/csrc/pl_context.h
@@ -194,6 +194,12 @@
   DevBuf<double> cls_table;
   int *cls_host_flag = nullptr;
   bool cls_ready = false;
+  DevBuf<unsigned long long> dcl_keys;
+  DevBuf<int> dcl_owner, dcl_dense_of_slot, dcl_flags;
+  DevBuf<uint16_t> dcl_slot;
+  int *dcl_host_flags = nullptr;
+  int dcl_fail_streak = 0, dcl_skip_left = 0;
+  bool dcl_pending = false;
   DevBuf<double> p2, small_scal, small_rc;
   bool small_use = false;
   bool persist_use = false;
diff --git a/pylatticedso_amd/csrc/pl_nodeword.h b/pylatticedso_amd/csrc/pl_nodeword.h
--- /dev/null
+++ b/pylatticedso_amd/csrc/pl_nodeword.h
@@ -0,0 +1,52 @@
+#pragma once
+#include <cmath>
+#include <cstddef>
+#include <cstdint>
+#include <cstring>
+#include <vector>
+
+namespace pl {
+
+constexpr int kRelByteMaxExp = 8;
+constexpr int kRelByteMaxMag = 127;
+
+inline bool same_bits(double a, double b) { return std::memcmp(&a, &b, sizeof(double)) == 0; }
+
+inline int rel_byte_exponent(const double *d, size_t n) {
+  int e = 0;
+  for (size_t i = 0; i < n; ++i) {
+    if (!std::isfinite(d[i])) return -1;
+    for (;;) {
+      const double s = std::ldexp(d[i], e);
+      if (std::fabs(s) > (double)kRelByteMaxMag) return -1;
+      if (s == std::floor(s)) break;
+      if (++e > kRelByteMaxExp) return -1;
+    }
+  }
+  for (size_t i = 0; i < n; ++i)
+    if (std::fabs(std::ldexp(d[i], e)) > (double)kRelByteMaxMag) return -1;
+  return e;
+}
+
+inline double rel_byte_value(int8_t b, int e) { return (double)b * std::ldexp(1.0, -e); }
+inline int8_t node_word_byte(uint32_t w, int k) { return (int8_t)(uint8_t)(w >> (8 * k)); }
+
+inline bool pack_rel_bytes(const double *d, size_t n_nodes, std::vector<uint32_t> &words, int &e_out) {
+  const int e = rel_byte_exponent(d, 3 * n_nodes);
+  if (e < 0) return false;
+  std::vector<uint32_t> w(n_nodes);
+  for (size_t i = 0; i < n_nodes; ++i) {
+    uint32_t word = 0;
+    for (int k = 0; k < 3; ++k) {
+      const int8_t b = (int8_t)(int)std::ldexp(d[3 * i + k], e);
+      if (!same_bits(rel_byte_value(b, e), d[3 * i + k])) return false;
+      word |= (uint32_t)(uint8_t)b << (8 * k);
+    }
+    w[i] = word;
+  }
+  words.swap(w);
+  e_out = e;
+  return true;
+}
+
+}
diff --git a/pylatticedso_amd/csrc/pl_solver.h b/pylatticedso_amd/csrc/pl_solver.h
--- a/pylatticedso_amd/csrc/pl_solver.h
+++ b/pylatticedso_amd/csrc/pl_solver.h
@@ -86,8 +86,13 @@
                      cs.rc, cs.tile_level ? (const double *)cs.Bt_inv : (const double *)nullptr, cs.yt,               \
                      useL ? (const int32_t *)cl.agg_of_tile.p : (const int32_t *)nullptr, cl.cen.p,                   \
                      (c->dist.active || useL) ? (const uint8_t *)c->sharedbits.p : (const uint8_t *)nullptr, cl.rc,   \
-                     cs.ncp, c->cond_use ? (const uint8_t *)c->cflag.p : (const uint8_t *)nullptr, cs.cm, rel32)
+                     cs.ncp, c->cond_use ? (const uint8_t *)c->cflag.p : (const uint8_t *)nullptr, cs.cm, rel32,   \
+                     nword, dtab, rscale)
   const float *rel32 = cs.rel_exact ? (const float *)cs.rel32.p : (const float *)nullptr;
+  const bool words = node_words_apply(c);
+  const uint32_t *dtab = words && cs.dcl_ready ? (const uint32_t *)cs.dcl_table : (const uint32_t *)nullptr;
+  const double rscale = words && cs.rel_e >= 0 ? std::ldexp(1.0, -cs.rel_e) : 0.0;
+  const uint32_t *nword = (dtab || rscale != 0.0) ? (const uint32_t *)cs.nword.p : (const uint32_t *)nullptr;
   if (useL) {
     if (tile_modes_now(c) == 12) PL_UPD(12, true, true);
     else PL_UPD(6, true, true);
@@ -112,7 +117,8 @@
                      c->hist.p, hist_slot, cs.rc, cs.ncp,                                                                \
                      useL ? (const int32_t *)cl.agg_of_tile.p : (const int32_t *)nullptr, cl.cen.p, cl.yc,                \
                      (c->dist.active || useL) ? (const uint8_t *)c->sharedbits.p : (const uint8_t *)nullptr, cl.rc,       \
-                     cl.ncp, c->cond_use ? (const uint8_t *)c->cflag.p : (const uint8_t *)nullptr, cs.cm, rel32)
+                     cl.ncp, c->cond_use ? (const uint8_t *)c->cflag.p : (const uint8_t *)nullptr, cs.cm, rel32,         \
+                     nword, dtab, rscale)
   const int64_t n_flat = c->cond_use ? c->N - c->n_cond : c->N;
 #define PL_DIRF(TM)                                                                                                      \
   hipLaunchKernelGGL((pl::k_pcg_direction_flat<PT, RT, TM>), dim3((unsigned)((3 * n_flat + pl::kBlock - 1) / pl::kBlock)), \
@@ -120,7 +126,8 @@
                      cs.agg_of_tile.p, cs.cen.p, cs.yc, cs.tile_level ? (const double *)cs.yt : (const double *)nullptr,  \
                      c->fixedbits.p, p, x, cur, nxt, c->hist.p, hist_slot, cs.rc, cs.ncp,                                \
                      c->cond_use ? (const int32_t *)c->ckeep.p : (const int32_t *)nullptr, cs.cm,                        \
-                     c->dist.active ? (const uint8_t *)c->sharedbits.p : (const uint8_t *)nullptr, rel32)
+                     c->dist.active ? (const uint8_t *)c->sharedbits.p : (const uint8_t *)nullptr, rel32, nword, dtab,   \
+                     rscale)
   if (!useL && sizeof(PT) == 8) {
     if (tile_modes_now(c) == 12) PL_DIRF(12);
     else PL_DIRF(6);
```

Result: faster. 256.8 million, median of 6 (+3.4%).
